# castacks/mvs_gi

Hardware: AMD Instinct MI355X
Metric: stereo frames/sec/GPU (G16V, 3-cam, D=16) + inv-dist L1 vs reference (higher is better)
Workload: dtype f16x3 (split-fp16 MFMA operands: 11 + 11 significant bits, f32 accumulate/activations)

## Files before the change

### include/mvsgi.h

```cpp
#ifndef MVSGI_H
#define MVSGI_H

#include <stddef.h>
#include <stdint.h>

#ifdef __cplusplus
extern "C" {
#endif

#define MVSGI_ABI_VERSION 8

typedef void* mvsgi_stream_t;

#define MVSGI_CONV_AUTO   0
#define MVSGI_CONV_DIRECT 1
#define MVSGI_CONV_MFMA   2
#define MVSGI_CONV_BF16X3 3
#define MVSGI_CONV_BF16X3_C16 4
#define MVSGI_CONV_BF16X3_V32 5
#define MVSGI_CONV_BF16X3_D32 6

#define MVSGI_CONV_F16 0x100

#define MVSGI_SPLIT_F16 1

int         mvsgi_abi_version(void);
const char* mvsgi_last_error(void);

#define MVSGI_SAT_SWEEP 1u
#define MVSGI_SAT_SPLIT 2u
#define MVSGI_SAT_WINO  4u
int mvsgi_saturation_flags(int clear, unsigned* flags);
int mvsgi_saturation_words(unsigned* words8);

int mvsgi_sweep_max_cams(void);
int mvsgi_sweep_std_f32(const float* feats, const float* grids, const void* grid_masks,
                        int grid_mask_is_f32, const float* masks, float* vol,
                        int B, int N, int C, int Hi, int Wi, int Hm, int Wm,
                        int D, int Ho, int Wo, mvsgi_stream_t stream);

int mvsgi_sweep_cat_f32(const float* feats, const float* grids, float* vol,
                        int B, int N, int C, int Hi, int Wi,
                        int D, int Ho, int Wo, mvsgi_stream_t stream);

int mvsgi_sweep_std_nhwc_f32(const float* feats, const float* grids, const void* grid_masks,
                             int grid_mask_is_f32, const float* masks, float* vol,
                             int B, int N, int C, int Hi, int Wi, int Hm, int Wm,
                             int D, int Ho, int Wo, mvsgi_stream_t stream);
int mvsgi_sweep_cat_nhwc_f32(const float* feats, const float* grids, float* vol,
                             int B, int N, int C, int Hi, int Wi,
                             int D, int Ho, int Wo, mvsgi_stream_t stream);

int mvsgi_sweep_validity_u8(const float* grids, const void* grid_masks, int grid_mask_is_f32,
                            const float* masks, unsigned char* vmask,
                            int B, int N, int Hm, int Wm, int D, int Ho, int Wo, mvsgi_stream_t stream);
int mvsgi_sweep_std_nhwc_valid_f32(const float* feats, const float* grids, const unsigned char* vmask,
                                   float* vol, int B, int N, int C, int Hi, int Wi,
                                   int D, int Ho, int Wo, mvsgi_stream_t stream);
int mvsgi_sweep_std_nhwc_valid_rig_f32(const float* feats, const float* grids, const unsigned char* vmask,
                                       float* vol, int B, int N, int C, int Hi, int Wi, int D, int Ho, int Wo,
                                       mvsgi_stream_t stream);

size_t mvsgi_conv3d_packed_weight_floats(int Cout, int Cin);
int mvsgi_conv3d_pack_weights_f32(const float* w_oidhw, float* w_packed, int Cout, int Cin,
                                  mvsgi_stream_t stream);
size_t mvsgi_conv3d_packed_weight_bytes_bf16x3(int Cout, int Cin);
int mvsgi_conv3d_pack_weights_bf16x3(const float* w_oidhw, void* w_packed, int Cout, int Cin,
                                     mvsgi_stream_t stream);
int mvsgi_conv3d_pack_weights_split(const float* w_oidhw, void* w_packed, int Cout, int Cin, int layout, mvsgi_stream_t stream);
int mvsgi_conv3d_f32(const float* x, const float* w_oidhw, const float* w_packed,
                     const float* scale, const float* shift, const float* res, float* y,
                     int B, int Cin, int Din, int Hin, int Win, int Cout,
                     int stride, float neg_slope, int impl, mvsgi_stream_t stream);
const char* mvsgi_conv3d_variant_f32(int B, int Cin, int Din, int Hin, int Win, int Cout,
                                     int stride, int impl);

int mvsgi_conv3d_up2_f32(const float* x, const void* w_packed, int w_layout ,
                         const float* scale, const float* shift, const float* res, float* y,
                         int B, int Cin, int Dl, int Hl, int Wl, int Cout, float neg_slope, mvsgi_stream_t stream);
const char* mvsgi_conv3d_up2_variant_f32(int B, int Cin, int Dl, int Hl, int Wl, int Cout, int w_layout);
int mvsgi_conv3d_v32_applies(int B, int Cin, int Din, int Hin, int Win, int Cout, int stride);
int mvsgi_conv3d_d32_applies(int B, int Cin, int Din, int Hin, int Win, int Cout, int stride);
int mvsgi_conv3d_up2_d32_applies(int B, int Cin, int Dl, int Hl, int Wl, int Cout);
size_t mvsgi_conv3d_packed_weight_bytes_bf16x3_v32(int Cout, int Cin);
int mvsgi_conv3d_pack_weights_bf16x3_v32(const float* w_oidhw, void* w_packed, int Cout, int Cin, mvsgi_stream_t stream);
size_t mvsgi_conv3d_packed_weight_bytes_bf16x3_c16(int Cin);
int mvsgi_conv3d_pack_weights_bf16x3_c16(const float* w_oidhw, void* w_packed, int Cin, mvsgi_stream_t stream);

size_t mvsgi_conv2d_packed_weight_floats(int Cout, int Cin);
int mvsgi_conv2d_pack_weights_f32(const float* w_oihw, float* w_packed, int Cout, int Cin,
                                  mvsgi_stream_t stream);
size_t mvsgi_conv2d_stem_packed_weight_bytes(void);
int mvsgi_conv2d_stem_pack_weights(const float* w_oihw, void* w_packed, mvsgi_stream_t stream);
size_t mvsgi_conv2d_packed_weight_bytes_bf16x3(int Cout, int Cin);
int mvsgi_conv2d_pack_weights_bf16x3(const float* w_oihw, void* w_packed, int Cout, int Cin,
                                     mvsgi_stream_t stream);
int mvsgi_conv2d_f32(const float* x, const float* w_oihw, const void* w_packed,
                     const float* scale, const float* shift, const float* res, float* y,
                     int B, int Cin, int Hin, int Win, int Cout, int ksize, int stride,
                     float neg_slope, int impl, int in_nchw, mvsgi_stream_t stream);
const char* mvsgi_conv2d_variant_f32(int Cin, int Cout, int ksize, int stride, int impl, int in_nchw);

int mvsgi_resize_trilinear_f32(const float* x, float* y, int B, int C,
                               int Di, int Hi, int Wi, int Do, int Ho, int Wo,
                               mvsgi_stream_t stream);

int mvsgi_softargmin_f32(const float* costs, const float* inv_idx, float* inv_dist,
                         float* norm_costs, int B, int D, int H, int W, int scale,
                         mvsgi_stream_t stream);

int mvsgi_softargmin_div_f32(const float* costs, const float* inv_idx, float* inv_dist,
                             float* norm_costs, int B, int D, int H, int W, int scale,
                             float post_div, mvsgi_stream_t stream);

#define MVSGI_SA_AUTO  0
#define MVSGI_SA_PIXEL 1
#define MVSGI_SA_BAND  2
int mvsgi_softargmin_scaled_f32(const float* costs, const float* inv_idx, float* inv_dist,
                                float* norm_costs, int B, int D, int H, int W, double scale,
                                int OH, int OW, float post_div, int variant, mvsgi_stream_t stream);

int mvsgi_confidence_f32(const float* costs, const float* inv_idx, float* max_prob, float* entropy,
                         float* spread, int* argmax, int B, int D, int H, int W, double scale,
                         int OH, int OW, float post_div, int normalize_entropy, mvsgi_stream_t stream);

int mvsgi_ncv_to_nvc_f32(const float* x, float* y, int B, int C, long long V, mvsgi_stream_t stream);
int mvsgi_nvc_to_ncv_f32(const float* x, float* y, int B, int C, long long V, mvsgi_stream_t stream);

int mvsgi_resblock2d_f32(const float* x, const void* w_packed1, const float* scale1, const float* shift1,
                         const void* w_packed2, const float* scale2, const float* shift2, float* y,
                         int N, int H, int W, float neg_slope, mvsgi_stream_t stream);

size_t mvsgi_split2d_bytes(int N, int H, int W);
int mvsgi_f32_to_split2d(const float* x, void* y_split, int N, int H, int W, mvsgi_stream_t stream);
int mvsgi_split2d_to_f32(const void* x_split, float* y, int N, int H, int W, mvsgi_stream_t stream);
size_t mvsgi_resblock2d_split_packed_weight_bytes(void);
int mvsgi_resblock2d_split_pack_weights(const float* w_oihw, const float* scale, void* w_packed, mvsgi_stream_t stream);
int mvsgi_resblock2d_split(const void* x_split, const void* w_packed1, const float* shift1,
                           const void* w_packed2, const float* shift2, void* y, int y_is_split,
                           int N, int H, int W, float neg_slope, mvsgi_stream_t stream);
int mvsgi_conv2d_s2_split(const void* x_split, const void* w_packed, const float* shift, void* y_split,
                          int N, int H, int W, float neg_slope, mvsgi_stream_t stream);
int mvsgi_conv2d_f32_out_split2d(const float* x, const float* w_oihw, const void* w_packed,
                                 const float* scale, const float* shift, const float* res, void* y_split,
                                 int B, int Cin, int Hin, int Win, int Cout, int ksize, int stride,
                                 float neg_slope, int impl, int in_nchw, mvsgi_stream_t stream);

int mvsgi_rays_panorama_f32(const float* dist, float* rays, int N, int H, int W,
                            float lat0, float lat1, float lon0, float lon1, mvsgi_stream_t stream);
int mvsgi_transform_points_f32(const float* T , const float* points, float* out,
                               int B, long long M, mvsgi_stream_t stream);
int mvsgi_grid_double_sphere_f32(const float* points, float* grid, unsigned char* mask, int B, long long M,
                                 float xi, float alpha, float fx, float fy, float cx, float cy,
                                 int calib_h, int calib_w, float w2, mvsgi_stream_t stream);
int mvsgi_grid_equirect_f32(const float* points, float* grid, int B, long long M, mvsgi_stream_t stream);
int mvsgi_rays_equirect_surrogate_f32(float* rays, int H, int W, mvsgi_stream_t stream);

int mvsgi_resample_bilinear_u8_f32(const unsigned char* imgs, const float* grid, const unsigned char* valid, float* out,
                                   long long M, int T, int Hr, int Wr, int H, int W, float invalid_value, mvsgi_stream_t stream);
int mvsgi_resample_bilinear_f32(const float* imgs, const float* grid, const unsigned char* valid, float* out, long long M, int T,
                                int C, int Hr, int Wr, int H, int W, float invalid_value, mvsgi_stream_t stream);
int mvsgi_resample_validity_u8(const float* grid, const unsigned char* ds_mask, unsigned char* valid, long long n,
                               mvsgi_stream_t stream);
int mvsgi_resample_u8_table_f32(float* table256);

int mvsgi_reproject_f32(const float* inv, const float* rays, const void* imgs, int img_kind, const float* T_host,
// ... 163 lines not shown
```

### mvs_gi_amd/_lib.py

```python
from __future__ import annotations

import ctypes
import os
from ctypes import c_char_p, c_double, c_float, c_int, c_longlong, c_size_t, c_void_p

_HERE = os.path.dirname(os.path.abspath(__file__))
LIB_PATH = os.environ.get("MVSGI_LIB", os.path.join(_HERE, "libmvsgi_hip.so"))

ABI_VERSION = 8


class MvsgiLibraryMissing(RuntimeError):
    pass


_P = c_void_p
SIGNATURES = {
    "mvsgi_abi_version": (c_int, []),
    "mvsgi_last_error": (c_char_p, []),
    "mvsgi_saturation_flags": (c_int, [c_int, _P]),
    "mvsgi_saturation_words": (c_int, [_P]),
    "mvsgi_sweep_max_cams": (c_int, []),
    "mvsgi_sweep_std_f32": (c_int, [_P, _P, _P, c_int, _P, _P] + [c_int] * 10 + [_P]),
    "mvsgi_sweep_cat_f32": (c_int, [_P, _P, _P] + [c_int] * 8 + [_P]),
    "mvsgi_sweep_std_nhwc_f32": (c_int, [_P, _P, _P, c_int, _P, _P] + [c_int] * 10 + [_P]),
    "mvsgi_sweep_cat_nhwc_f32": (c_int, [_P, _P, _P] + [c_int] * 8 + [_P]),
    "mvsgi_sweep_validity_u8": (c_int, [_P, _P, c_int, _P, _P] + [c_int] * 7 + [_P]),
    "mvsgi_sweep_std_nhwc_valid_f32": (c_int, [_P, _P, _P, _P] + [c_int] * 8 + [_P]),
    "mvsgi_sweep_std_nhwc_valid_split": (c_int, [_P, _P, _P, _P] + [c_int] * 9 + [_P]),
    "mvsgi_sweep_std_nhwc_valid_rig_f32": (c_int, [_P, _P, _P, _P] + [c_int] * 8 + [_P]),
    "mvsgi_conv3d_packed_weight_floats": (c_size_t, [c_int, c_int]),
    "mvsgi_conv3d_pack_weights_f32": (c_int, [_P, _P, c_int, c_int, _P]),
    "mvsgi_conv3d_packed_weight_bytes_bf16x3": (c_size_t, [c_int, c_int]),
    "mvsgi_conv3d_pack_weights_bf16x3": (c_int, [_P, _P, c_int, c_int, _P]),
    "mvsgi_conv3d_pack_weights_split": (c_int, [_P, _P, c_int, c_int, c_int, _P]),
    "mvsgi_conv3d_f32": (c_int, [_P] * 7 + [c_int] * 7 + [c_float, c_int, _P]),
    "mvsgi_conv3d_variant_f32": (c_char_p, [c_int] * 8),
    "mvsgi_conv3d_up2_f32": (c_int, [_P, _P, c_int] + [_P] * 4 + [c_int] * 6 + [c_float, _P]),
    "mvsgi_conv3d_up2_variant_f32": (c_char_p, [c_int] * 7),
    "mvsgi_conv3d_v32_applies": (c_int, [c_int] * 7),
    "mvsgi_conv3d_d32_applies": (c_int, [c_int] * 7),
    "mvsgi_conv3d_up2_d32_applies": (c_int, [c_int] * 6),
    "mvsgi_conv3d_packed_weight_bytes_bf16x3_v32": (c_size_t, [c_int, c_int]),
    "mvsgi_conv3d_pack_weights_bf16x3_v32": (c_int, [_P, _P, c_int, c_int, _P]),
    "mvsgi_conv3d_packed_weight_bytes_bf16x3_c16": (c_size_t, [c_int]),
    "mvsgi_conv3d_pack_weights_bf16x3_c16": (c_int, [_P, _P, c_int, _P]),
    "mvsgi_conv2d_stem_packed_weight_bytes": (c_size_t, []),
    "mvsgi_conv2d_stem_pack_weights": (c_int, [_P, _P, _P]),
    "mvsgi_conv2d_packed_weight_floats": (c_size_t, [c_int, c_int]),
    "mvsgi_conv2d_pack_weights_f32": (c_int, [_P, _P, c_int, c_int, _P]),
    "mvsgi_conv2d_packed_weight_bytes_bf16x3": (c_size_t, [c_int, c_int]),
    "mvsgi_conv2d_pack_weights_bf16x3": (c_int, [_P, _P, c_int, c_int, _P]),
    "mvsgi_conv2d_f32": (c_int, [_P] * 7 + [c_int] * 7 + [c_float, c_int, c_int, _P]),
    "mvsgi_conv2d_variant_f32": (c_char_p, [c_int] * 6),
    "mvsgi_resblock2d_f32": (c_int, [_P] * 8 + [c_int] * 3 + [c_float, _P]),
    "mvsgi_split2d_bytes": (c_size_t, [c_int] * 3),
    "mvsgi_f32_to_split2d": (c_int, [_P, _P] + [c_int] * 3 + [_P]),
    "mvsgi_split2d_to_f32": (c_int, [_P, _P] + [c_int] * 3 + [_P]),
    "mvsgi_resblock2d_split_packed_weight_bytes": (c_size_t, []),
    "mvsgi_resblock2d_split_pack_weights": (c_int, [_P, _P, _P, _P]),
    "mvsgi_resblock2d_split": (c_int, [_P] * 6 + [c_int] * 4 + [c_float, _P]),
    "mvsgi_conv2d_s2_split": (c_int, [_P] * 4 + [c_int] * 3 + [c_float, _P]),
    "mvsgi_conv2d_f32_out_split2d": (c_int, [_P] * 7 + [c_int] * 7 + [c_float, c_int, c_int, _P]),
    "mvsgi_resize_trilinear_f32": (c_int, [_P, _P] + [c_int] * 8 + [_P]),
    "mvsgi_softargmin_f32": (c_int, [_P, _P, _P, _P] + [c_int] * 5 + [_P]),
    "mvsgi_softargmin_div_f32": (c_int, [_P, _P, _P, _P] + [c_int] * 5 + [c_float, _P]),
    "mvsgi_softargmin_scaled_f32": (c_int, [_P, _P, _P, _P] + [c_int] * 4 + [c_double, c_int, c_int, c_float, c_int, _P]),
    "mvsgi_confidence_f32": (c_int, [_P] * 6 + [c_int] * 4 + [c_double, c_int, c_int, c_float, c_int, _P]),
    "mvsgi_rays_panorama_f32": (c_int, [_P, _P, c_int, c_int, c_int] + [c_float] * 4 + [_P]),
    "mvsgi_transform_points_f32": (c_int, [_P, _P, _P, c_int, c_longlong, _P]),
    "mvsgi_grid_double_sphere_f32": (c_int, [_P, _P, _P, c_int, c_longlong] + [c_float] * 6 + [c_int, c_int, c_float, _P]),
    "mvsgi_grid_equirect_f32": (c_int, [_P, _P, c_int, c_longlong, _P]),
    "mvsgi_rays_equirect_surrogate_f32": (c_int, [_P, c_int, c_int, _P]),
    "mvsgi_resample_bilinear_u8_f32": (c_int, [_P, _P, _P, _P, c_longlong] + [c_int] * 5 + [c_float, _P]),
    "mvsgi_resample_bilinear_f32": (c_int, [_P, _P, _P, _P, c_longlong] + [c_int] * 6 + [c_float, _P]),
    "mvsgi_resample_validity_u8": (c_int, [_P, _P, _P, c_longlong, _P]),
    "mvsgi_resample_u8_table_f32": (c_int, [_P]),
    "mvsgi_reproject_f32": (c_int, [_P, _P, _P, c_int] + [_P] * 6 + [c_longlong] + [c_int] * 6 + [c_float, c_float, _P]),
    "mvsgi_deform_conv2d_pack_weights_f32": (c_int, [_P, _P] + [c_int] * 4 + [_P]),
    "mvsgi_deform_conv2d_f32": (c_int, [_P, _P, c_int] + [_P] * 5 + [c_int] * 13 + [c_float, _P]),
    "mvsgi_act_split_bytes": (c_size_t, [c_int] * 5),
    "mvsgi_act_f32_to_split": (c_int, [_P, _P] + [c_int] * 5 + [_P]),
    "mvsgi_act_split_to_f32": (c_int, [_P, _P] + [c_int] * 5 + [_P]),
    "mvsgi_conv3d_f32_out_split": (c_int, [_P] * 6 + [c_int] * 7 + [c_float, _P]),
    "mvsgi_conv3d_rs16_split": (c_int, [_P] * 5 + [c_int] * 4 + [c_float, _P]),
    "mvsgi_conv3d_rs16_split_out_split": (c_int, [_P] * 5 + [c_int] * 4 + [c_float, _P]),
    "mvsgi_conv3d_s2rs_packed_weight_bytes": (c_size_t, []),
    "mvsgi_conv3d_s2rs_pack_weights": (c_int, [_P, _P, _P, _P]),
    "mvsgi_conv3d_s2rs": (c_int, [_P] * 4 + [c_int] * 4 + [c_float, _P]),
    "mvsgi_conv3d_rs_packed_weight_bytes": (c_size_t, [c_int, c_int]),
    "mvsgi_conv3d_rs_pack_weights": (c_int, [_P, _P, c_int, c_int, _P]),
    "mvsgi_conv3d_rs_split": (c_int, [_P] * 6 + [c_int] * 7 + [c_float, _P]),
    "mvsgi_conv3d_up2_f32_out_split": (c_int, [_P, _P, c_int] + [_P] * 4 + [c_int] * 6 + [c_float, _P]),
    "mvsgi_conv3d_up2_poly_split": (c_int, [_P] * 5 + [c_int] * 4 + [c_float, _P]),
    "mvsgi_conv3d_head_split_packed_weight_bytes": (c_size_t, [c_int]),
    "mvsgi_conv3d_head_split_pack_weights": (c_int, [_P, _P, c_int, _P]),
    "mvsgi_conv3d_head_split": (c_int, [_P, _P, c_float, c_float, _P] + [c_int] * 5 + [c_float, _P]),
    "mvsgi_conv3d_head_split_pack_weights_f16": (c_int, [_P, _P, c_int, _P]),
    "mvsgi_conv3d_head_split_f16": (c_int, [_P, _P, c_float, c_float, _P] + [c_int] * 5 + [c_float, _P]),
    "mvsgi_conv3d_head_rec32_f16": (c_int, [_P, _P, c_float, c_float, _P] + [c_int] * 5 + [c_float, _P]),
    "mvsgi_conv3d_up2_poly_rec32": (c_int, [_P] * 5 + [c_int] * 4 + [c_float, _P]),
    "mvsgi_conv3d_up2_poly_plan_bytes": (c_size_t, [c_int] * 3),
    "mvsgi_conv3d_up2_poly_plan": (c_int, [_P, _P] + [c_int] * 3),
    "mvsgi_conv3d_up2_poly_f32": (c_int, [_P] * 5 + [c_int] * 4 + [c_float, _P]),
    "mvsgi_act_f32_to_split_fmt": (c_int, [_P, _P] + [c_int] * 6 + [_P]),
    "mvsgi_act_split_to_f32_fmt": (c_int, [_P, _P] + [c_int] * 6 + [_P]),
    "mvsgi_sweep_std_nhwc_valid_split_fmt": (c_int, [_P, _P, _P, _P] + [c_int] * 10 + [_P]),
    "mvsgi_conv3d_f32_out_split_fmt": (c_int, [_P] * 6 + [c_int] * 7 + [c_float, c_int, _P]),
    "mvsgi_conv3d_rs_pack_weights_fmt": (c_int, [_P, _P, c_int, c_int, c_int, _P]),
    "mvsgi_conv3d_rs_split_fmt": (c_int, [_P] * 6 + [c_int] * 7 + [c_float, c_int, _P]),
    "mvsgi_conv3d_rs16_split_fmt": (c_int, [_P] * 5 + [c_int] * 5 + [c_float, c_int, _P]),
    "mvsgi_conv3d_s2rs_pack_weights_fmt": (c_int, [_P, _P, _P, c_int, _P]),
    "mvsgi_conv3d_s2rs_fmt": (c_int, [_P] * 4 + [c_int] * 4 + [c_float, c_float, c_int, _P]),
    "mvsgi_conv3d_s2rs_out_fmt": (c_int, [_P] * 4 + [c_int] * 4 + [c_float, c_float, c_int, c_int, _P]),
    "mvsgi_conv3d_up2_poly_plan_fmt": (c_int, [_P, _P] + [c_int] * 4),
    "mvsgi_conv3d_wino32_packed_weight_bytes": (c_size_t, []),
    "mvsgi_conv3d_wino32_applies": (c_int, [c_int] * 6 + [c_float]),
    "mvsgi_conv3d_wino32_pack_weights": (c_int, [_P] * 4),
    "mvsgi_conv3d_wino32_f16": (c_int, [_P] * 6 + [c_int] * 6 + [c_float, _P]),
    "mvsgi_conv3d_up2_poly_fmt": (c_int, [_P] * 5 + [c_int] * 5 + [c_float, c_int, _P]),
    "mvsgi_conv3d_up2_poly_wino_pays": (c_int, [c_int] * 4),
    "mvsgi_ncv_to_nvc_f32": (c_int, [_P, _P, c_int, c_int, c_longlong, _P]),
    "mvsgi_nvc_to_ncv_f32": (c_int, [_P, _P, c_int, c_int, c_longlong, _P]),
    "mvsgi_instance_norm_ws_bytes": (c_size_t, [c_int] * 3),
    "mvsgi_instance_norm_f32": (c_int, [_P] * 6 + [c_int] * 3 + [c_float, c_float, _P]),
# ... 60 lines not shown
```

### mvs_gi_amd/csrc/conv3d.hip

```cpp
#include "common.hpp"
#include "conv_common.hpp"
#include "conv3d_variants.hpp"
#ifdef MVSGI_STAMPS
#include <cstdio>
#include <cstdlib>
#endif

namespace {

__global__ void pack_head_weights_kernel(const float* __restrict__ w, float* __restrict__ wp, int Cin) {
    const int idx = blockIdx.x * 256 + threadIdx.x;
    if (idx >= 27 * Cin) return;
    const int tap = idx / Cin, ci = idx % Cin;
    wp[idx] = w[ci * 27 + tap];
}

#include "conv3d_f32mfma.hpp"
#include "conv3d_bf16x3.hpp"


__global__ __launch_bounds__(256) void conv3d_head_kernel(ConvArgs a, int dchunk, int nd) {
    constexpr int TH = 8, TW = 32, ITH = TH + 2, ITW = TW + 2, PV = ITH * ITW;
    constexpr int NT = (PV + 31) / 32;
    constexpr int TPW = (NT + 3) / 4;
// ... 139 lines not shown
__global__ __launch_bounds__(256) void conv3d_direct_kernel(ConvArgs a) {
    const int groups = (a.Cout + CO - 1) / CO;
    const long long total = (long long)a.B * a.Do * a.Ho * a.Wo * groups;
    const long long idx = (long long)blockIdx.x * 256 + threadIdx.x;
    if (idx >= total) return;
    const int cg = (int)(idx % groups);
    const long long vox = idx / groups;
    const int ow = (int)(vox % a.Wo);
    const int oh = (int)((vox / a.Wo) % a.Ho);
    const int od = (int)((vox / ((long long)a.Wo * a.Ho)) % a.Do);
    const int b = (int)(vox / ((long long)a.Wo * a.Ho * a.Do));
    const int co0 = cg * CO;
    float acc[CO];
#pragma unroll
    for (int o = 0; o < CO; ++o) acc[o] = 0.f;
    for (int kd = 0; kd < 3; ++kd) {
        const int id = od * a.stride - 1 + kd;
        if (id < 0 || id >= a.Din) continue;
        for (int kh = 0; kh < 3; ++kh) {
            const int ih = oh * a.stride - 1 + kh;
            if (ih < 0 || ih >= a.Hin) continue;
            for (int kw = 0; kw < 3; ++kw) {
                const int iw = ow * a.stride - 1 + kw;
                if (iw < 0 || iw >= a.Win) continue;
                const int tap = (kd * 3 + kh) * 3 + kw;
                const float* xp = a.x + ((((long long)b * a.Din + id) * a.Hin + ih) * a.Win + iw) * a.Cin;
                for (int ci = 0; ci < a.Cin; ++ci) {
                    const float xv = xp[ci];
#pragma unroll
                    for (int o = 0; o < CO; ++o) {
                        const int co = co0 + o;
                        if (co < a.Cout) acc[o] = fmaf(xv, a.w_oidhw[((long long)co * a.Cin + ci) * 27 + tap], acc[o]);
                    }
                }
            }
        }
    }
#pragma unroll
    for (int o = 0; o < CO; ++o) {
        const int co = co0 + o;
        if (co >= a.Cout) break;
        float r = acc[o] * a.scale[co] + a.shift[co];
        if (a.res) r += a.res[vox * a.Cout + co];
        r = r > 0.f ? r : r * a.neg_slope;
        a.y[vox * a.Cout + co] = r;
    }
}

int launch_head(ConvArgs a, hipStream_t st) {
    constexpr size_t lds_bytes = (size_t)27 * 360 * sizeof(float);
    a.tiles_h = (int)mvsgi::cdiv(a.Ho, 8);
    a.tiles_w = (int)mvsgi::cdiv(a.Wo, 32);
    const long long windows = (long long)a.B * a.tiles_h * a.tiles_w;
    long long nd = windows >= 1024 ? 1 : mvsgi::cdiv(1024, windows);
    if (nd > mvsgi::cdiv(a.Do, 2)) nd = mvsgi::cdiv(a.Do, 2);
    const int dchunk = (int)mvsgi::cdiv(a.Do, nd);
    nd = mvsgi::cdiv(a.Do, dchunk);
    a.tiles_d = (int)nd;
    const long long nt = windows * nd;
    MVSGI_REQUIRE(nt < (1ll << 31), "conv3d: too many tiles");
    MVSGI_REQUIRE((long long)a.Hin * a.Win * a.Cin < (1ll << 31), "conv3d(head): plane too large for 32-bit offsets");
    hipLaunchKernelGGL(conv3d_head_kernel, dim3((unsigned)nt), dim3(256), lds_bytes, st, a, dchunk, (int)nd);
    return mvsgi::check_launch("mvsgi_conv3d_f32(head)");
}

int launch_direct(const ConvArgs& a, hipStream_t st) {
    const long long vox = (long long)a.B * a.Do * a.Ho * a.Wo;
    if (a.Cout == 1) {
        hipLaunchKernelGGL((conv3d_direct_kernel<1>), dim3((unsigned)mvsgi::cdiv(vox, 256)), dim3(256), 0, st, a);
    } else {
        const long long total = vox * mvsgi::cdiv(a.Cout, 4);
        hipLaunchKernelGGL((conv3d_direct_kernel<4>), dim3((unsigned)mvsgi::cdiv(total, 256)), dim3(256), 0, st, a);
    }
    return mvsgi::check_launch("mvsgi_conv3d_f32(direct)");
}

bool v32_applies(const ConvArgs& a) {
    if (a.Cout % 32 || a.Cin % 16 || a.stride != 1) return false;
    const long long big = (long long)a.B * mvsgi::cdiv(a.Do, 4) * mvsgi::cdiv(a.Ho, 4) * mvsgi::cdiv(a.Wo, 16);
    const long long mid = (long long)a.B * mvsgi::cdiv(a.Do, 2) * mvsgi::cdiv(a.Ho, 4) * mvsgi::cdiv(a.Wo, 16);
    return a.Cout == 32 ? big >= 384 : mid * mvsgi::cdiv(a.Cout, 64) >= 384;
}

int select_variant_up2(const ConvArgs& a, int w_layout) {
    if (w_layout == MVSGI_CONV_BF16X3_D32) {
        const int base = a.Cin % 32 ? V_COUNT : select_variant_up2(a, MVSGI_CONV_BF16X3);
        const bool d2 = a.Do == 2;
        if (base == B3U_N64) return d2 ? B3DU2_N64 : B3DU_N64;
        if (base == B3U_N96) return d2 ? B3DU2_N96 : B3DU_N96;
        mvsgi::fail("mvsgi_conv3d_up2_f32: the 32-channel-slice kernels do not apply to this problem (see mvsgi_conv3d_up2_d32_applies)");
        return V_COUNT;
    }
    const bool c16_layout = w_layout == MVSGI_CONV_BF16X3_C16;
    if (w_layout == MVSGI_CONV_BF16X3_V32) {
        if (!v32_applies(a) || !a.wp) { mvsgi::fail("mvsgi_conv3d_up2_f32: the 32x32x16 kernel does not apply to this problem"); return V_COUNT; }
        return a.Cout == 32 ? B3VU_N32 : B3VU_N64;
    }
    if (a.Cin % 16 || a.Cout % 16) {
        mvsgi::fail("mvsgi_conv3d_up2_f32: Cin, Cout must be multiples of 16 (got %d, %d)", a.Cin, a.Cout);
        return V_COUNT;
    }
    if (!a.wp) { mvsgi::fail("mvsgi_conv3d_up2_f32: needs w_packed (bf16x3 layout)"); return V_COUNT; }
    const int CT = a.Cout / 16;
    const long long big = (long long)a.B * mvsgi::cdiv(a.Do, 4) * mvsgi::cdiv(a.Ho, 4) * mvsgi::cdiv(a.Wo, 16);
    const long long mid = (long long)a.B * mvsgi::cdiv(a.Do, 2) * mvsgi::cdiv(a.Ho, 4) * mvsgi::cdiv(a.Wo, 16);
    if (CT == 1) return c16_layout ? B3PU_N16 : B3U_N16;
    if (CT == 2) {
        if (big >= 384) return B3U_N32;
        const long long cus = mvsgi::device_cus(), r32 = mvsgi::cdiv(big, cus), rm = mvsgi::cdiv(mid, cus);
        return 157 * (100 + 85 * (r32 - 1)) < 100 * (100 + 85 * (rm - 1)) ? B3U_N32 : B3U_N32_M;
    }
    if (CT == 3) return B3U_N48;
    if (CT % 6 == 0 && mid * (CT / 6) >= 384) return B3U_N96;
    if (CT % 2 == 0 && (long long)a.B * mvsgi::cdiv(a.Do, 2) * mvsgi::cdiv(a.Ho, 2) * mvsgi::cdiv(a.Wo, 16) * (CT / 2) <= mvsgi::device_cus())
        return B3U_N32_TB;
    return B3U_N64;
}

int select_variant(const ConvArgs& a, int impl);

int d32_variant(const ConvArgs& a) {
    if (a.stride != 1 || a.Cin % 32 || a.Cout % 16) return V_COUNT;
    ConvArgs b = a;
    static const float dummy = 0.f;
    if (!b.wp) b.wp = reinterpret_cast<const f32x4*>(&dummy);
    const bool d2 = a.Do == 2;
    switch (select_variant(b, MVSGI_CONV_BF16X3)) {
        case B3_N64: return d2 ? B3D2_N64 : B3D_N64;
        case B3_N64_H5: return d2 ? B3D2_N64_H5 : B3D_N64_H5;
        case B3_N64_W8: return d2 ? B3D2_N64_W8 : B3D_N64_W8;
        case B3_N96: return d2 ? B3D2_N96 : B3D_N96;
        case B3_N96_H5: return d2 ? B3D2_N96_H5 : B3D_N96_H5;
        case B3_N96_W8: return d2 ? B3D2_N96_W8 : B3D_N96_W8;
        case B3_N128_P: return B3D_N128_P;
        case B3_N128_PH5: return B3D_N128_PH5;
        case B3_N128_PW8: return B3D_N128_PW8;
        case B3_N192_PH5: return B3D_N192_PH5;
        case B3_N192_PW8: return B3D_N192_PW8;
        case B3_N16_TW: return d2 && a.Cout % 32 == 0 ? B3D2_N32_TB : V_COUNT;
        case B3_N32_TB: return d2 ? B3D2_N32_TB : B3D_N32_TB;
        case B3_N64_S: return d2 ? B3D2_N64_S : B3D_N64_S;
        default: return V_COUNT;
    }
}

int select_variant(const ConvArgs& a, int impl) {
    const bool mfma_ok = (a.Cin % 16 == 0) && (a.Cout % 16 == 0);
    const bool head_ok = (a.Cout == 1) && (a.Cin % 16 == 0) && (a.stride == 1);
    if (impl == MVSGI_CONV_BF16X3_C16) {
        if (a.Cout != 16 || a.Cin % 16 || a.stride != 1) {
            mvsgi::fail("mvsgi_conv3d_f32: the Cout == 16 plane kernel needs Cout == 16, Cin %% 16 == 0, stride 1 (got %d, %d, %d)",
                        a.Cout, a.Cin, a.stride);
            return V_COUNT;
        }
        if (!a.wp) { mvsgi::fail("mvsgi_conv3d_f32: tiled path needs w_packed"); return V_COUNT; }
        return B3P_N16;
    }
    if (impl == MVSGI_CONV_BF16X3_V32) {
        if (!v32_applies(a)) {
            mvsgi::fail("mvsgi_conv3d_f32: the 32x32x16 kernel does not apply to this problem (see mvsgi_conv3d_v32_applies)");
            return V_COUNT;
        }
        if (!a.wp) { mvsgi::fail("mvsgi_conv3d_f32: tiled path needs w_packed"); return V_COUNT; }
        return a.Cout == 32 ? B3V_N32 : B3V_N64;
    }
    if (impl == MVSGI_CONV_BF16X3_D32) {
        const int v = d32_variant(a);
// ... 12 lines not shown
        return V_COUNT;
    }
    if (!a.wp) { mvsgi::fail("mvsgi_conv3d_f32: tiled path needs w_packed"); return V_COUNT; }
    if (head_ok && impl == MVSGI_CONV_MFMA) return V_HEAD;
    if (!mfma_ok) {
        mvsgi::fail("mvsgi_conv3d_f32: MFMA path needs Cin, Cout multiples of 16 (got %d, %d)", a.Cin, a.Cout);
        return V_COUNT;
    }
    const int CT = a.Cout / 16;
    const long long vox = (long long)a.B * a.Do * a.Ho * a.Wo;
    if (impl == MVSGI_CONV_BF16X3) {
        if (a.stride == 2) {
            const long long s2bricks = (long long)a.B * mvsgi::cdiv(a.Do, 2) * mvsgi::cdiv(a.Ho, 4) * mvsgi::cdiv(a.Wo, 8);
            if (CT % 12 == 0 && s2bricks * (CT / 12) >= 512) return B3_S2_N192;
            if (CT % 8 == 0 && s2bricks * (CT / 8) >= 512) return B3_S2_N128;
            if (CT % 6 == 0 && s2bricks * (CT / 6) >= 512) return B3_S2_N96;
            if (CT <= 3 || s2bricks * mvsgi::cdiv(CT, 2) <= mvsgi::device_cus()) return B3_S2_N32B;
            return B3_S2_N64;
        }
        const long long big = (long long)a.B * mvsgi::cdiv(a.Do, 4) * mvsgi::cdiv(a.Ho, 4) * mvsgi::cdiv(a.Wo, 16);
        const long long mid = (long long)a.B * mvsgi::cdiv(a.Do, 2) * mvsgi::cdiv(a.Ho, 4) * mvsgi::cdiv(a.Wo, 16);
        if (CT == 1) return B3_N16;
        if (CT == 2) return big >= 384 ? B3_N32 : B3_N32_TB;
        if (CT == 3) return B3_N48;
        const bool h5ok = a.Ho % 5 == 0 && a.Ho % 4 != 0;
        const bool w8 = a.Ho % 10 == 0 && a.Wo % 16 == 8;
        if (a.Do == 1 && CT >= 8 && CT % 4 == 0) {
            const long long rows5 = (long long)a.B * (a.Ho / 5) * mvsgi::cdiv(a.Wo, 16);
            if (h5ok && CT % 12 == 0 && rows5 * (CT / 12) >= 384) return w8 ? B3_N192_PW8 : B3_N192_PH5;
            if (h5ok && CT % 8 == 0 && rows5 * (CT / 8) >= mvsgi::device_cus() / 2) return w8 ? B3_N128_PW8 : B3_N128_PH5;
            if (CT % 8 == 0 && (long long)a.B * mvsgi::cdiv(a.Ho, 4) * mvsgi::cdiv(a.Wo, 16) * (CT / 8) >= 384) return B3_N128_P;
        }
        if (CT % 6 == 0 && h5ok &&
            (long long)a.B * mvsgi::cdiv(a.Do, 2) * (a.Ho / 5) * mvsgi::cdiv(a.Wo, 16) * (CT / 6) >= 384) return w8 ? B3_N96_W8 : B3_N96_H5;
        if (CT % 6 == 0 && mid * (CT / 6) >= 384) return B3_N96;
        const long long cus = mvsgi::device_cus();
        if (CT % 4 == 0 && CT % 6 != 0 && mid * (CT / 4) < 4 * cus) {
            const long long tiny = (long long)a.B * a.Do * mvsgi::cdiv(a.Ho, 4) * mvsgi::cdiv(a.Wo, 16);
            if (tiny * CT <= cus) return B3_N16_TW;
            const long long slices = a.Cin / 16;
            struct Cand { int v; long long units, a_ns, b_ns; };
            const Cand cand[] = {
                {B3_N32_TB, tiny * (CT / 2), 5700, 1000},
                {B3_N64_S, tiny * (CT / 4), 6600, 1700},
                {B3_N64, mid * (CT / 4), 8700, 2600},
                {w8 ? B3_N64_W8 : B3_N64_H5, a.Ho % 5 ? 0 : (long long)a.B * mvsgi::cdiv(a.Do, 2) * (CT / 4) *
                                                 (w8 ? (a.Ho / 10) * (a.Wo / 8) : (a.Ho / 5) * mvsgi::cdiv(a.Wo, 16)), 8400, 3500},
            };
            int best = B3_N64;
            long long best_cost = -1;
            for (const Cand& c : cand) {
                if (c.units <= 0) continue;
                const long long rounds = mvsgi::cdiv(c.units, cus);
                const long long cost = (c.a_ns + c.b_ns * slices) * (100 + 85 * (rounds - 1));
                if (best_cost < 0 || cost < best_cost) { best_cost = cost; best = c.v; }
            }
            return best;
        }
        if (h5ok && (long long)a.B * mvsgi::cdiv(a.Do, 2) * (a.Ho / 5) * mvsgi::cdiv(a.Wo, 16) * mvsgi::cdiv(CT, 4) >= 384)
            return w8 ? B3_N64_W8 : B3_N64_H5;
        if (mid * mvsgi::cdiv(CT, 4) >= 384) return B3_N64;
        const long long tiny = (long long)a.B * a.Do * mvsgi::cdiv(a.Ho, 4) * mvsgi::cdiv(a.Wo, 16);
        if (tiny * CT <= cus) return B3_N16_TW;
        const long long rounds32 = mvsgi::cdiv(tiny * mvsgi::cdiv(CT, 2), cus), rounds64 = mvsgi::cdiv(tiny * mvsgi::cdiv(CT, 4), cus);
        return 2 * rounds32 <= 3 * rounds64 ? B3_N32_TB : B3_N64_S;
    }
    if (a.stride == 1) {
        if (CT == 1) return V_S1_N16_B256;
        if (CT <= 3) return vox >= 256ll * 512 ? V_S1_N32_B256 : V_S1_N32_B64;
        return vox * CT >= 128ll * 4 * 1024 ? V_S1_N64_B128 : V_S1_N64_B64;
    }
    return CT <= 3 ? V_S2_N32_B64 : V_S2_N64_B64;
}

int launch_variant(int v, const ConvArgs& a, hipStream_t st) {
    if (a.f16) return mvsgi::conv3d_launch_b3_f16(v, &a, st);
    switch (v) {
        case V_DIRECT1:
        case V_DIRECT4: return launch_direct(a, st);
        case V_HEAD: return launch_head(a, st);
#define MVSGI_MFMA(V, ...) case V: return launch_mfma<__VA_ARGS__>(a, st);
#define MVSGI_B3(V, K, ...) case V: return MVSGI_B3_LAUNCH##K(false, __VA_ARGS__)(a, st);
#include "conv3d_variants.inc"
#undef MVSGI_MFMA
#undef MVSGI_B3
    }
    return mvsgi::fail("mvsgi_conv3d_f32: bad variant %d", v);
}

int fill_args(ConvArgs& a, const float* x, const float* w_oidhw, const float* w_packed, const float* scale,
              const float* shift, const float* res, float* y, int B, int Cin, int Din, int Hin, int Win, int Cout,
              int stride, float neg_slope) {
    MVSGI_REQUIRE(B > 0 && Cin > 0 && Cout > 0 && Din > 0 && Hin > 0 && Win > 0, "mvsgi_conv3d_f32: bad dims");
    MVSGI_REQUIRE(stride == 1 || stride == 2, "mvsgi_conv3d_f32: stride %d not in {1, 2}", stride);
    a.x = x;
    a.w_oidhw = w_oidhw;
    a.wp = reinterpret_cast<const f32x4*>(w_packed);
    a.scale = scale;
    a.shift = shift;
    a.res = res;
    a.y = y;
    a.B = B;
    a.Cin = Cin;
    a.Din = Din;
    a.Hin = Hin;
    a.Win = Win;
    a.Cout = Cout;
    a.stride = stride;
    a.neg_slope = neg_slope;
    a.Do = (Din - 1) / stride + 1;
    a.Ho = (Hin - 1) / stride + 1;
    a.Wo = (Win - 1) / stride + 1;
    return 0;
}

int split_flag(ConvArgs& a, int& impl, const char* who) {
    a.f16 = (impl & MVSGI_CONV_F16) != 0;
    impl &= ~MVSGI_CONV_F16;
    MVSGI_REQUIRE(!a.f16 || impl == MVSGI_CONV_BF16X3 || impl == MVSGI_CONV_BF16X3_C16 || impl == MVSGI_CONV_BF16X3_V32 || impl == MVSGI_CONV_BF16X3_D32,
                  "%s: MVSGI_CONV_F16 goes with MVSGI_CONV_BF16X3 / _C16 / _V32 (got %d)", who, impl);
    MVSGI_REQUIRE(!a.f16 || (a.Cin % 16 == 0 && a.Cout % 16 == 0), "%s: the fp16 split needs Cin, Cout multiples of 16 (got %d, %d)", who, a.Cin, a.Cout);
    return 0;
}

const char* variant_name(int v, const ConvArgs& a) {
    switch (v) {
        case V_DIRECT1: return "conv3d_direct_kernel<1>";
        case V_DIRECT4: return "conv3d_direct_kernel<4>";
        case V_HEAD: return "conv3d_head_kernel";
#define MVSGI_MFMA(V, ...) case V: return "conv3d_mfma_kernel<" #__VA_ARGS__ ">";
#define MVSGI_B3(V, K, ...) case V: return a.f16 ? "conv3d_f16x3" #K "<" #__VA_ARGS__ ">" : "conv3d_bf16x3" #K "<" #__VA_ARGS__ ">";
#include "conv3d_variants.inc"
#undef MVSGI_MFMA
#undef MVSGI_B3
    }
    return nullptr;
}

}

extern "C" size_t mvsgi_conv3d_packed_weight_floats(int Cout, int Cin) {
    return (size_t)27 * (size_t)Cout * (size_t)Cin;
}

extern "C" size_t mvsgi_conv3d_packed_weight_bytes_bf16x3(int Cout, int Cin) {
    return (size_t)(Cin / 16) * pairs_of(3) * (size_t)(Cout / 16) * 2 * 64 * 16;
}

extern "C" int mvsgi_conv3d_pack_weights_bf16x3(const float* w_oidhw, void* w_packed, int Cout, int Cin,
                                                mvsgi_stream_t stream) {
    MVSGI_REQUIRE(w_oidhw && w_packed, "mvsgi_conv3d_pack_weights_bf16x3: null pointer");
    MVSGI_REQUIRE(Cout > 0 && Cin > 0 && Cout % 16 == 0 && Cin % 16 == 0,
                  "mvsgi_conv3d_pack_weights_bf16x3: Cout=%d Cin=%d must be positive multiples of 16", Cout, Cin);
    const long long total = (long long)(Cin / 16) * pairs_of(3) * (Cout / 16) * 64;
    hipLaunchKernelGGL(pack_weights_bf16x3_kernel, dim3((unsigned)mvsgi::cdiv(total, 256)), dim3(256), 0,
                       mvsgi::as_stream(stream), w_oidhw, reinterpret_cast<bf16x8*>(w_packed), Cout, Cin, 27, false);
    return mvsgi::check_launch("mvsgi_conv3d_pack_weights_bf16x3");
}

extern "C" int mvsgi_conv3d_pack_weights_split(const float* w_oidhw, void* w_packed, int Cout, int Cin, int layout,
                                               mvsgi_stream_t stream) {
    MVSGI_REQUIRE(w_oidhw && w_packed, "mvsgi_conv3d_pack_weights_split: null pointer");
    const bool f16 = (layout & MVSGI_CONV_F16) != 0;
    layout &= ~MVSGI_CONV_F16;
    MVSGI_REQUIRE(Cout > 0 && Cin > 0 && Cout % 16 == 0 && Cin % 16 == 0,
                  "mvsgi_conv3d_pack_weights_split: Cout=%d Cin=%d must be positive multiples of 16", Cout, Cin);
    bf16x8* wp = reinterpret_cast<bf16x8*>(w_packed);
    if (layout == MVSGI_CONV_BF16X3) {
        const long long total = (long long)(Cin / 16) * pairs_of(3) * (Cout / 16) * 64;
        hipLaunchKernelGGL(pack_weights_bf16x3_kernel, dim3((unsigned)mvsgi::cdiv(total, 256)), dim3(256), 0, mvsgi::as_stream(stream),
                           w_oidhw, wp, Cout, Cin, 27, f16);
    } else if (layout == MVSGI_CONV_BF16X3_C16) {
        MVSGI_REQUIRE(Cout == 16, "mvsgi_conv3d_pack_weights_split: the plane layout is for Cout == 16 (got %d)", Cout);
        const int total = (Cin / 16) * 5 * 3 * 64;
        hipLaunchKernelGGL(pack_weights_bf16x3_c16_kernel, dim3((unsigned)mvsgi::cdiv(total, 256)), dim3(256), 0, mvsgi::as_stream(stream),
                           w_oidhw, wp, Cin, f16);
    } else if (layout == MVSGI_CONV_BF16X3_V32) {
        MVSGI_REQUIRE(Cout % 32 == 0, "mvsgi_conv3d_pack_weights_split: the 32x32x16 layout needs Cout %% 32 == 0 (got %d)", Cout);
        const long long total = (long long)(Cin / 16) * (Cout / 32) * 27 * 64;
        hipLaunchKernelGGL(pack_weights_bf16x3_v32_kernel, dim3((unsigned)mvsgi::cdiv(total, 256)), dim3(256), 0, mvsgi::as_stream(stream),
                           w_oidhw, wp, Cout, Cin, f16);
    } else if (layout == MVSGI_CONV_BF16X3_D32) {
        MVSGI_REQUIRE(Cin % 32 == 0, "mvsgi_conv3d_pack_weights_split: the 32-channel-slice layout needs Cin %% 32 == 0 (got %d)", Cin);
        const long long total = (long long)(Cin / 32) * (Cout / 16) * 27 * 64;
        const size_t used = (size_t)total * 2 * sizeof(bf16x8), all = mvsgi_conv3d_packed_weight_bytes_bf16x3(Cout, Cin);
        MVSGI_REQUIRE(used <= all && hipMemsetAsync(reinterpret_cast<char*>(w_packed) + used, 0, all - used, mvsgi::as_stream(stream)) == hipSuccess,
                      "mvsgi_conv3d_pack_weights_split: clearing the unused tail of the 32-channel-slice layout failed");
        hipLaunchKernelGGL(pack_weights_bf16x3_d32_kernel, dim3((unsigned)mvsgi::cdiv(total, 256)), dim3(256), 0, mvsgi::as_stream(stream),
                           w_oidhw, wp, Cout, Cin, f16);
    } else {
        return mvsgi::fail("mvsgi_conv3d_pack_weights_split: layout %d is not a split-kernel layout", layout);
    }
    return mvsgi::check_launch("mvsgi_conv3d_pack_weights_split");
}

extern "C" size_t mvsgi_conv3d_packed_weight_bytes_bf16x3_v32(int Cout, int Cin) {
    return (size_t)(Cin / 16) * (Cout / 32) * 27 * 2 * 64 * 16;
}

extern "C" int mvsgi_conv3d_pack_weights_bf16x3_v32(const float* w_oidhw, void* w_packed, int Cout, int Cin,
                                                    mvsgi_stream_t stream) {
    MVSGI_REQUIRE(w_oidhw && w_packed, "mvsgi_conv3d_pack_weights_bf16x3_v32: null pointer");
    MVSGI_REQUIRE(Cout > 0 && Cin > 0 && Cout % 32 == 0 && Cin % 16 == 0,
                  "mvsgi_conv3d_pack_weights_bf16x3_v32: Cout=%d must be a multiple of 32, Cin=%d of 16", Cout, Cin);
    const long long total = (long long)(Cin / 16) * (Cout / 32) * 27 * 64;
    hipLaunchKernelGGL(pack_weights_bf16x3_v32_kernel, dim3((unsigned)mvsgi::cdiv(total, 256)), dim3(256), 0,
                       mvsgi::as_stream(stream), w_oidhw, reinterpret_cast<bf16x8*>(w_packed), Cout, Cin, false);
    return mvsgi::check_launch("mvsgi_conv3d_pack_weights_bf16x3_v32");
}

extern "C" int mvsgi_conv3d_d32_applies(int B, int Cin, int Din, int Hin, int Win, int Cout, int stride) {
    ConvArgs a{};
    static const float dummy = 0.f;
    if (fill_args(a, &dummy, &dummy, &dummy, &dummy, &dummy, nullptr, nullptr, B, Cin, Din, Hin, Win, Cout, stride, 1.f))
        return 0;
    return d32_variant(a) != V_COUNT ? 1 : 0;
}

extern "C" int mvsgi_conv3d_v32_applies(int B, int Cin, int Din, int Hin, int Win, int Cout, int stride) {
    ConvArgs a{};
    static const float dummy = 0.f;
    if (fill_args(a, &dummy, &dummy, &dummy, &dummy, &dummy, nullptr, nullptr, B, Cin, Din, Hin, Win, Cout, stride, 1.f))
        return 0;
    return v32_applies(a) ? 1 : 0;
}

extern "C" size_t mvsgi_conv3d_packed_weight_bytes_bf16x3_c16(int Cin) { return (size_t)(Cin / 16) * 5 * 3 * 2 * 64 * 16; }

extern "C" int mvsgi_conv3d_pack_weights_bf16x3_c16(const float* w_oidhw, void* w_packed, int Cin, mvsgi_stream_t stream) {
    MVSGI_REQUIRE(w_oidhw && w_packed, "mvsgi_conv3d_pack_weights_bf16x3_c16: null pointer");
    MVSGI_REQUIRE(Cin > 0 && Cin % 16 == 0, "mvsgi_conv3d_pack_weights_bf16x3_c16: Cin=%d must be a positive multiple of 16", Cin);
    const int total = (Cin / 16) * 5 * 3 * 64;
    hipLaunchKernelGGL(pack_weights_bf16x3_c16_kernel, dim3((unsigned)mvsgi::cdiv(total, 256)), dim3(256), 0,
                       mvsgi::as_stream(stream), w_oidhw, reinterpret_cast<bf16x8*>(w_packed), Cin, false);
    return mvsgi::check_launch("mvsgi_conv3d_pack_weights_bf16x3_c16");
}

extern "C" int mvsgi_conv3d_pack_weights_f32(const float* w_oidhw, float* w_packed, int Cout, int Cin,
                                             mvsgi_stream_t stream) {
    MVSGI_REQUIRE(w_oidhw && w_packed, "mvsgi_conv3d_pack_weights_f32: null pointer");
    if (Cout == 1 && Cin > 0 && Cin % 16 == 0) {
        hipLaunchKernelGGL(pack_head_weights_kernel, dim3((unsigned)mvsgi::cdiv(27 * Cin, 256)), dim3(256), 0,
                           mvsgi::as_stream(stream), w_oidhw, w_packed, Cin);
        return mvsgi::check_launch("mvsgi_conv3d_pack_weights_f32");
    }
    MVSGI_REQUIRE(Cout > 0 && Cin > 0 && Cout % 16 == 0 && Cin % 16 == 0,
                  "mvsgi_conv3d_pack_weights_f32: Cout=%d Cin=%d must be positive multiples of 16 (or Cout == 1)",
                  Cout, Cin);
    const long long total = (long long)(Cin / 16) * 27 * (Cout / 16) * 64;
    hipLaunchKernelGGL(pack_weights_kernel, dim3((unsigned)mvsgi::cdiv(total, 256)), dim3(256), 0,
                       mvsgi::as_stream(stream), w_oidhw, reinterpret_cast<f32x4*>(w_packed), Cout, Cin, 27);
    return mvsgi::check_launch("mvsgi_conv3d_pack_weights_f32");
}

extern "C" int mvsgi_conv3d_f32(const float* x, const float* w_oidhw, const float* w_packed, const float* scale,
                                const float* shift, const float* res, float* y, int B, int Cin, int Din, int Hin,
                                int Win, int Cout, int stride, float neg_slope, int impl, mvsgi_stream_t stream) {
    MVSGI_REQUIRE(x && y && scale && shift, "mvsgi_conv3d_f32: null pointer");
    ConvArgs a{};
    if (fill_args(a, x, w_oidhw, w_packed, scale, shift, res, y, B, Cin, Din, Hin, Win, Cout, stride, neg_slope))
        return 1;
    if (split_flag(a, impl, "mvsgi_conv3d_f32")) return 1;
    const int v = select_variant(a, impl);
    if (v == V_COUNT) return 1;
    return launch_variant(v, a, mvsgi::as_stream(stream));
}

extern "C" int mvsgi_conv3d_f32_out_split_fmt(const float* x, const float* w_packed_b3, const float* scale, const float* shift,
                                              const float* res, void* y_split, int B, int Cin, int Din, int Hin, int Win, int Cout,
                                              int stride, float neg_slope, int fmt, mvsgi_stream_t stream) {
    MVSGI_REQUIRE(fmt == 0 || fmt == MVSGI_SPLIT_F16, "mvsgi_conv3d_f32_out_split: fmt %d not in {0, MVSGI_SPLIT_F16}", fmt);
    MVSGI_REQUIRE(x && y_split && scale && shift && w_packed_b3, "mvsgi_conv3d_f32_out_split: null pointer");
    MVSGI_REQUIRE(Cin % 16 == 0 && Cout % 16 == 0, "mvsgi_conv3d_f32_out_split: Cin, Cout must be multiples of 16");
    ConvArgs a{};
    if (fill_args(a, x, nullptr, w_packed_b3, scale, shift, res, reinterpret_cast<float*>(y_split), B, Cin, Din, Hin, Win, Cout,
                  stride, neg_slope))
        return 1;
    a.y_split = static_cast<unsigned char*>(y_split);
    a.f16 = fmt != 0;
    const int v = select_variant(a, MVSGI_CONV_BF16X3);
    if (v == V_COUNT) return 1;
    return launch_variant(v, a, mvsgi::as_stream(stream));
}
extern "C" int mvsgi_conv3d_f32_out_split(const float* x, const float* w_packed_b3, const float* scale, const float* shift,
                                          const float* res, void* y_split, int B, int Cin, int Din, int Hin, int Win, int Cout,
                                          int stride, float neg_slope, mvsgi_stream_t stream) {
    return mvsgi_conv3d_f32_out_split_fmt(x, w_packed_b3, scale, shift, res, y_split, B, Cin, Din, Hin, Win, Cout, stride, neg_slope, 0, stream);
}

extern "C" const char* mvsgi_conv3d_variant_f32(int B, int Cin, int Din, int Hin, int Win, int Cout, int stride,
                                                int impl) {
    ConvArgs a{};
    static const float dummy = 0.f;
    if (fill_args(a, &dummy, &dummy, &dummy, &dummy, &dummy, nullptr, nullptr, B, Cin, Din, Hin, Win, Cout, stride,
                  1.f))
        return nullptr;
    if (split_flag(a, impl, "mvsgi_conv3d_variant_f32")) return nullptr;
    const int v = select_variant(a, impl);
    return variant_name(v, a);
}

extern "C" int mvsgi_conv3d_up2_f32(const float* x, const void* w_packed, int w_layout, const float* scale,
                                    const float* shift, const float* res, float* y, int B, int Cin, int Dl, int Hl,
                                    int Wl, int Cout, float neg_slope, mvsgi_stream_t stream) {
    const bool f16 = (w_layout & MVSGI_CONV_F16) != 0;
    w_layout &= ~MVSGI_CONV_F16;
    MVSGI_REQUIRE(w_layout == MVSGI_CONV_BF16X3 || (w_layout == MVSGI_CONV_BF16X3_C16 && Cout == 16) ||
                      (w_layout == MVSGI_CONV_BF16X3_V32 && Cout % 32 == 0) || (w_layout == MVSGI_CONV_BF16X3_D32 && Cin % 32 == 0),
                  "mvsgi_conv3d_up2_f32: w_layout %d not valid for Cout %d", w_layout, Cout);
    MVSGI_REQUIRE(x && y && scale && shift && w_packed, "mvsgi_conv3d_up2_f32: null pointer");
    MVSGI_REQUIRE(Dl > 0 && Hl > 0 && Wl > 0 && Dl < (1 << 20) && Hl < (1 << 20) && Wl < (1 << 20),
                  "mvsgi_conv3d_up2_f32: bad dims");
    ConvArgs a{};
    if (fill_args(a, x, nullptr, static_cast<const float*>(w_packed), scale, shift, res, y, B, Cin, 2 * Dl, 2 * Hl,
                  2 * Wl, Cout, 1, neg_slope))
        return 1;
    a.f16 = f16;
    const int v = select_variant_up2(a, w_layout);
    if (v == V_COUNT) return 1;
    return launch_variant(v, a, mvsgi::as_stream(stream));
}

extern "C" int mvsgi_conv3d_up2_f32_out_split(const float* x, const void* w_packed, int w_layout, const float* scale, const float* shift,
                                              const float* res, void* y_split, int B, int Cin, int Dl, int Hl, int Wl, int Cout,
                                              float neg_slope, mvsgi_stream_t stream) {
    const bool f16 = (w_layout & MVSGI_CONV_F16) != 0;
    w_layout &= ~MVSGI_CONV_F16;
    MVSGI_REQUIRE(w_layout == MVSGI_CONV_BF16X3 || (w_layout == MVSGI_CONV_BF16X3_C16 && Cout == 16),
                  "mvsgi_conv3d_up2_f32_out_split: w_layout %d not valid for Cout %d", w_layout, Cout);
    MVSGI_REQUIRE(x && y_split && scale && shift && w_packed, "mvsgi_conv3d_up2_f32_out_split: null pointer");
    MVSGI_REQUIRE(Dl > 0 && Hl > 0 && Wl > 0 && Dl < (1 << 20) && Hl < (1 << 20) && Wl < (1 << 20),
                  "mvsgi_conv3d_up2_f32_out_split: bad dims");
    ConvArgs a{};
    if (fill_args(a, x, nullptr, static_cast<const float*>(w_packed), scale, shift, res, reinterpret_cast<float*>(y_split), B, Cin,
                  2 * Dl, 2 * Hl, 2 * Wl, Cout, 1, neg_slope))
        return 1;
    a.y_split = static_cast<unsigned char*>(y_split);
    a.f16 = f16;
    const int v = select_variant_up2(a, w_layout);
    if (v == V_COUNT) return 1;
    return launch_variant(v, a, mvsgi::as_stream(stream));
}

extern "C" int mvsgi_conv3d_up2_d32_applies(int B, int Cin, int Dl, int Hl, int Wl, int Cout) {
    ConvArgs a{};
    static const float dummy = 0.f;
    if (Cin % 32 || Cout % 16 || Dl <= 0 || Hl <= 0 || Wl <= 0 ||
        fill_args(a, &dummy, nullptr, &dummy, &dummy, &dummy, nullptr, nullptr, B, Cin, 2 * Dl, 2 * Hl, 2 * Wl, Cout, 1, 1.f))
        return 0;
    const int base = select_variant_up2(a, MVSGI_CONV_BF16X3);
    return (base == B3U_N64 || base == B3U_N96) ? 1 : 0;
}

extern "C" const char* mvsgi_conv3d_up2_variant_f32(int B, int Cin, int Dl, int Hl, int Wl, int Cout, int w_layout) {
    ConvArgs a{};
    static const float dummy = 0.f;
    if (fill_args(a, &dummy, nullptr, &dummy, &dummy, &dummy, nullptr, nullptr, B, Cin, 2 * Dl, 2 * Hl, 2 * Wl, Cout, 1,
                  1.f))
        return nullptr;
    a.f16 = (w_layout & MVSGI_CONV_F16) != 0;
    const int v = select_variant_up2(a, w_layout & ~MVSGI_CONV_F16);
    return variant_name(v, a);
}
```

### mvs_gi_amd/csrc/conv3d_bf16x3.hpp

```cpp
#pragma once
#ifndef MVSGI_ABL
#define MVSGI_ABL 0
#endif

#include "split_fmt.hpp"

constexpr int kVSB = 80;

__device__ __forceinline__ void split_bf16x4(const f32x4 x, u32x2& hi, u32x2& lo) {
#pragma unroll
    for (int p = 0; p < 2; ++p) {
        const f32x2 v = {x[2 * p], x[2 * p + 1]};
        const unsigned hb = __builtin_bit_cast(unsigned, __builtin_convertvector(v, bf16x2));
        const f32x2 hf = {__builtin_bit_cast(float, hb << 16), __builtin_bit_cast(float, hb & 0xffff0000u)};
        hi[p] = hb;
        float r0 = v[0] - hf[0], r1 = v[1] - hf[1];
        asm volatile("" : "+v"(r0));
        asm volatile("" : "+v"(r1));
        lo[p] = __builtin_bit_cast(unsigned, __builtin_convertvector(f32x2{r0, r1}, bf16x2));
    }
}
__device__ __forceinline__ f32x4 fma4(const f32x4 a, const f32x4 b, const f32x4 c) {
    f32x4 r;
#pragma unroll
// ... 81 lines not shown
    const long long o = ((((long long)cc * CT + ct) * kPairs + p) * 2) * 64 + lane;
    wp[o] = __builtin_bit_cast(bf16x8, hi);
    wp[o + 64] = __builtin_bit_cast(bf16x8, lo);
}

__global__ void pack_weights_bf16x3_d32_kernel(const float* __restrict__ w, bf16x8* __restrict__ wp, int Cout, int Cin, bool f16 = false) {
    const int CT = Cout / 16;
    const long long total = (long long)(Cin / 32) * CT * 27 * 64;
    const long long idx = (long long)blockIdx.x * 256 + threadIdx.x;
    if (idx >= total) return;
    const int lane = (int)(idx & 63);
    long long r = idx >> 6;
    const int tap = (int)(r % 27);
    r /= 27;
    const int ct = (int)(r % CT);
    const int cc = (int)(r / CT);
    const int kg = lane >> 4;
    const int co = ct * 16 + (lane & 15);
    const int ci = (2 * cc + (kg & 1)) * 16 + (kg >> 1) * 8;
    u16x8 hi, lo;
    for (int j = 0; j < 8; ++j) {
        unsigned short h_, l_;
        split_weight(w[((long long)co * Cin + ci + j) * 27 + tap], f16, h_, l_);
        hi[j] = h_;
        lo[j] = l_;
    }
    const long long o = ((((long long)cc * CT + ct) * 27 + tap) * 2) * 64 + lane;
    wp[o] = __builtin_bit_cast(bf16x8, hi);
    wp[o + 64] = __builtin_bit_cast(bf16x8, lo);
}

__global__ void pack_weights_bf16x3_c16_kernel(const float* __restrict__ w, bf16x8* __restrict__ wp, int Cin, bool f16 = false) {
    const int total = (Cin / 16) * 5 * 3 * 64;
    const int idx = blockIdx.x * 256 + threadIdx.x;
    if (idx >= total) return;
    const int lane = idx & 63;
    int r = idx >> 6;
    const int kd = r % 3;
    r /= 3;
    const int p = r % 5;
    const int cc = r / 5;
    const int kg = lane >> 4, co = lane & 15;
    const int ci = cc * 16 + (kg >> 1) * 8;
    const int t2 = 2 * p + (kg & 1);
    u16x8 hi, lo;
    for (int j = 0; j < 8; ++j) {
        const float v = t2 < 9 ? w[((long long)co * Cin + ci + j) * 27 + kd * 9 + t2] : 0.f;
        unsigned short h_, l_;
        split_weight(v, f16, h_, l_);
        hi[j] = h_;
        lo[j] = l_;
    }
    const long long o = ((long long)((cc * 5 + p) * 3 + kd) * 2) * 64 + lane;
    wp[o] = __builtin_bit_cast(bf16x8, hi);
    wp[o + 64] = __builtin_bit_cast(bf16x8, lo);
}

__global__ void pack_weights_bf16x3_v32_kernel(const float* __restrict__ w, bf16x8* __restrict__ wp, int Cout, int Cin, bool f16 = false) {
    const int CT = Cout / 32;
    const long long total = (long long)(Cin / 16) * CT * 27 * 64;
    const long long idx = (long long)blockIdx.x * 256 + threadIdx.x;
    if (idx >= total) return;
    const int lane = (int)(idx & 63);
    long long r = idx >> 6;
    const int tap = (int)(r % 27);
    r /= 27;
    const int ct = (int)(r % CT);
    const int cc = (int)(r / CT);
    const int co = ct * 32 + (lane & 31);
    const int ci = cc * 16 + (lane >> 5) * 8;
    u16x8 hi, lo;
    for (int j = 0; j < 8; ++j) {
        const float v = w[((long long)co * Cin + ci + j) * 27 + tap];
        unsigned short h_, l_;
        split_weight(v, f16, h_, l_);
        hi[j] = h_;
        lo[j] = l_;
    }
    const long long o = ((((long long)cc * CT + ct) * 27 + tap) * 2) * 64 + lane;
    wp[o] = __builtin_bit_cast(bf16x8, hi);
    wp[o + 64] = __builtin_bit_cast(bf16x8, lo);
}

template <int NW, int MW, int WM, int WN, int TD, int TH, int TW, int S, int KD, bool UPS, bool PLANE, bool V32, bool WLDS, bool F16, bool D32 = false, int DK = 3, int BRD = 0>
__device__ __forceinline__ void conv3d_x3_body(const ConvArgs& a) {
    static_assert(!WLDS || (WN == 1 && KD == 3 && !UPS && !PLANE && !V32 && S == 1 && NW == 1 && MW <= 2), "LDS-staged weights: one shared cout tile, one or two voxel tiles per wave");
    static_assert(!V32 || (S == 1 && KD == 3 && TW == 16 && TH % 2 == 0 && !PLANE), "32x32x16 schedule: stride 1, 16-wide even bricks");
    static_assert(!PLANE || (NW == 1 && WN == 1 && WM == 4 && TH == 4 && MW == TD && TW == 16 && S == 1 && KD == 3),
                  "plane schedule: Cout == 16, 4 h-rows x TD planes x 16 w per brick");
    static_assert(!UPS || (S == 1 && KD == 3 && TD % 2 == 0 && TH % 2 == 0 && TW % 2 == 0),
                  "fused upsample: stride 1, even bricks (halo bricks are whole 2x2x2 cells)");
    static_assert(WM * WN == 4, "4 consumer waves per workgroup");
    static_assert(WM * MW * (V32 ? 32 : 16) == TD * TH * TW, "brick must be covered by the voxel tiles");
    static_assert(KD == 3 || (KD == 1 && TD == 1), "2-D bricks are one plane thick");
    constexpr int SD = KD == 1 ? 1 : S;
    static_assert(!D32 || (KD == 3 && S == 1 && !PLANE && !V32 && !WLDS), "32-channel slices: stride-1 3x3x3 variants (plain or fused upsample) only");
    static_assert(DK == 3 || (D32 && DK >= 1 && (TD == 1 ? DK <= 2 : (TD == 2 && WM == 2 && MW * 16 == TH * TW))), "depth skip: one- or two-plane bricks whose waves own whole planes");
    constexpr bool DKU = D32 && TD == 1 && DK == 2;
    constexpr int kTaps = KD * 9, kPairs = D32 ? 9 * DK : pairs_of(KD);
    constexpr int kWBlk = D32 ? 27 : kPairs;
    constexpr int ITD = (TD - 1) * SD + KD, ITH = (TH - 1) * S + 3, ITW = (TW - 1) * S + 3;
    constexpr int IV = ITD * ITH * ITW;
    constexpr int QB = D32 ? 3 : 2;
    constexpr int NIT = (IV * (1 << QB) + 255) / 256;
    constexpr int ROWP = V32 ? ((ITW * kVSB + 255) / 256) * 256 : ITW * kVSB;
    constexpr int SUB = ITD * ITH * ROWP;
    constexpr int BUF = D32 ? 2 * SUB : SUB;
    constexpr int WB = WLDS ? (MW * NW == 1 ? 8 : 4) :
                       (KD == 3 && !PLANE && !V32 && MW * NW == 1) ? 16 : (KD == 3 && !PLANE && !V32 && MW * NW == 2) ? 8 :
                       (KD == 3 && !PLANE && !V32 && NW == 2 && MW == 4) ? 5 :
                       NW <= 2 ? 4 : 2;
    constexpr int LA = WB - 1;
    constexpr int NSLOT = ((kPairs + WB - 1) / WB) * WB;
    static_assert(NSLOT % WB == 0 && NSLOT >= kPairs, "pipeline geometry");
    constexpr bool RPRE = MW * NW <= 8;
#ifndef MVSGI_WARM
#define MVSGI_WARM 0
#endif
    constexpr bool WARM = MVSGI_WARM && KD == 3 && !UPS && !PLANE && !V32 && !WLDS && S == 1 && MW * NW <= 2;

    constexpr int WBYTES = WLDS ? NW * kPairs * 2048 : 0;
    constexpr int BUFW = BUF + WBYTES;
    constexpr int WARM_LDS = 2 * BUFW;
    extern __shared__ __attribute__((aligned(16))) unsigned char ldsb[];
    float satm = 0.f;

    const int tid = threadIdx.x, lane = tid & 63;
    const int wave = __builtin_amdgcn_readfirstlane(tid >> 6);
    const bool producer = wave >= 4;
    const int CT = a.Cout / (V32 ? 32 : 16);
    const int ny = (CT + WN * NW - 1) / (WN * NW);
    const int nchunks = a.Cin / (D32 ? 32 : 16);
    const int total = a.total_units;
    const int G = gridDim.x;
    const int nmine = (total - (int)blockIdx.x + G - 1) / G;
    const int U = nmine * nchunks;
#ifdef MVSGI_STAMPS
    int nst = 0;
#define STAMP()                                                                                     \
    if (a.dbg && blockIdx.x == 8 && nst < 120) {                                                    \
        unsigned long long t_;                                                                      \
        asm volatile("s_memtime %0\n\ts_waitcnt lgkmcnt(0)" : "=s"(t_)::"memory");                  \
        if (lane == 0) a.dbg[wave * 128 + nst] = t_;                                                \
        nst++;                                                                                      \
    }
#else
#define STAMP()
#endif
    STAMP()

#define MVSGI_DECODE_DH(T, OD, OH, B) { OD = (T % a.tiles_d) * TD + a.od_off; T /= a.tiles_d; OH = (T % a.tiles_h) * TH; B = T / a.tiles_h; }
#define MVSGI_DECODE(ID, CB, B, OD, OH, OW)                       \
    {                                                             \
        int t_ = xcd_remap((ID), total);                          \
        CB = t_ % ny;                                             \
        t_ /= ny;                                                 \
        OW = (t_ % a.tiles_w) * TW;                               \
        t_ /= a.tiles_w;                                          \
        MVSGI_DECODE_DH(t_, OD, OH, B)                            \
    }

    if (producer) {
        const int ptid = tid - 256;
        if constexpr (UPS) {
            constexpr int CD = ITD / 2, CH = ITH / 2, CW = ITW / 2, NC = CD * CH * CW;
            constexpr int NCQ = NC << QB;
            constexpr int NITU = (NCQ + 255) / 256;
            constexpr int RF = NCQ / 256, REM = NCQ - RF * 256;
            constexpr bool HALF = REM > 0 && 2 * REM <= 256;
#define MVSGI_UPS_CQ(IT) ((HALF && (IT) == RF) ? RF * 256 + (ptid >> 1) : ptid + (IT) * 256)
#define MVSGI_UPS_LIVE(IT) ((HALF && (IT) == RF) ? (ptid >> 1) < REM : ptid + (IT) * 256 < NCQ)
            const int Dl = a.Din >> 1, Hl = a.Hin >> 1, Wl = a.Win >> 1;
            const int sH_ = Wl * a.Cin, sD_ = Hl * sH_;
            int lo_d[NITU], lo_h[NITU], lo_w[NITU];
            unsigned inmask[NITU];
            const float* xb = a.x;
            f32x4 crA[NITU][8], crB[NITU][8];
            unsigned imA[NITU], imB[NITU];
#define MVSGI_PLAN_UPS(UNIT)                                                                            \
            {                                                                                           \
                int cb_, b_, od_, oh_, ow_;                                                             \
                MVSGI_DECODE(UNIT, cb_, b_, od_, oh_, ow_)                                              \
                (void)cb_;                                                                              \
                _Pragma("unroll") for (int it = 0; it < NITU; ++it) {                                   \
                    const int c = MVSGI_UPS_CQ(it) >> QB;                                               \
                    const int cw = c % CW, ch = (c / CW) % CH, cd = c / (CW * CH);                      \
                    const int gd = od_ - 1 + 2 * cd, gh = oh_ - 1 + 2 * ch, gw = ow_ - 1 + 2 * cw;      \
                    lo_d[it] = (gd - 1) >> 1;                                                           \
                    lo_h[it] = (gh - 1) >> 1;                                                           \
                    lo_w[it] = (gw - 1) >> 1;                                                           \
                    inmask[it] = (gd >= 0 && gd < a.Din ? 1u : 0u) | (gd + 1 < a.Din ? 2u : 0u) |       \
                                 (gh >= 0 && gh < a.Hin ? 4u : 0u) | (gh + 1 < a.Hin ? 8u : 0u) |       \
                                 (gw >= 0 && gw < a.Win ? 16u : 0u) | (gw + 1 < a.Win ? 32u : 0u);      \
                }                                                                                       \
                xb = a.x + (long long)b_ * Dl * Hl * Wl * a.Cin;                                        \
            }
#define MVSGI_CLAMP(V, N) ((V) < 0 ? 0 : ((V) > (N) - 1 ? (N) - 1 : (V)))
            int k2 = 0, cc2 = 0;
#define MVSGI_ISSUE_UPS_BEGIN()                                                                         \
            if (cc2 == 0 && k2 > 0) { MVSGI_PLAN_UPS((int)blockIdx.x + k2 * G) }
#define MVSGI_ISSUE_UPS1(CR, IM, IT)                                                                    \
            {                                                                                           \
                const int q = MVSGI_UPS_CQ(IT) & ((1 << QB) - 1);                                       \
                const bool live = MVSGI_UPS_LIVE(IT);                                                   \
                const int d0 = live ? MVSGI_CLAMP(lo_d[IT], Dl) : 0, d1 = live ? MVSGI_CLAMP(lo_d[IT] + 1, Dl) : 0; \
                const int h0 = live ? MVSGI_CLAMP(lo_h[IT], Hl) : 0, h1 = live ? MVSGI_CLAMP(lo_h[IT] + 1, Hl) : 0; \
                const int w0 = live ? MVSGI_CLAMP(lo_w[IT], Wl) : 0, w1 = live ? MVSGI_CLAMP(lo_w[IT] + 1, Wl) : 0; \
                const int cofs = cc2 * (D32 ? 32 : 16) + q * 4;                                         \
                 \
                const int od_[2] = {__mul24(d0, sD_), __mul24(d1, sD_)}, oh_[2] = {__mul24(h0, sH_), __mul24(h1, sH_)};   \
                const int ow_[2] = {__mul24(w0, a.Cin) + cofs, __mul24(w1, a.Cin) + cofs};              \
                _Pragma("unroll") for (int k = 0; k < 8; ++k)                                           \
                    CR[IT][k] = *reinterpret_cast<const f32x4*>(xb + (od_[(k >> 2) & 1] + oh_[(k >> 1) & 1] + ow_[k & 1])); \
                IM[IT] = inmask[IT];                                                                    \
            }
#define MVSGI_ISSUE_UPS_END()                                                                           \
            {                                                                                           \
                if (++cc2 == nchunks) { cc2 = 0; ++k2; }                                                \
                if (k2 >= nmine) { k2 = nmine - 1; cc2 = nchunks - 1; }                                 \
            }
#define MVSGI_ISSUE_UPS(CR, IM)                                                                         \
            {                                                                                           \
                MVSGI_ISSUE_UPS_BEGIN()                                                                 \
                _Pragma("unroll") for (int it = 0; it < NITU; ++it) MVSGI_ISSUE_UPS1(CR, IM, it)        \
                MVSGI_ISSUE_UPS_END()                                                                   \
            }
#define MVSGI_LERP2(A, B, O0, O1)    \
            {                                                                                           \
                const f32x4 d_ = fma4((A), f32x4{-1.f, -1.f, -1.f, -1.f}, (B));    \
                O0 = fma4(d_, f32x4{0.25f, 0.25f, 0.25f, 0.25f}, (A));             \
                O1 = fma4(d_, f32x4{0.75f, 0.75f, 0.75f, 0.75f}, (A));             \
            }
#define MVSGI_PUT_UPS1(CR, IM, DST, IT)                                                                 \
            if (HALF && (IT) == RF) {                                                                   \
                 \
                if (MVSGI_UPS_LIVE(IT)) {                                                               \
                    const int cq_ = MVSGI_UPS_CQ(IT), c = cq_ >> QB, q = cq_ & 3, kd = ptid & 1;        \
                    const int sub_ = D32 ? ((cq_ >> 2) & 1) * SUB : 0;                                  \
                    const int cw = c % CW, ch = (c / CW) % CH, cd = c / (CW * CH);                      \
                    const float f_ = kd ? 0.75f : 0.25f;                                                \
                    const f32x4 f4_ = {f_, f_, f_, f_};                                                 \
                    f32x4 xd[2][2], xh[2][2], xo[2][2];                                                 \
                    _Pragma("unroll") for (int j = 0; j < 4; ++j) {                                     \
                        const f32x4 d_ = fma4(CR[IT][j], f32x4{-1.f, -1.f, -1.f, -1.f}, CR[IT][4 + j]); \
                        xd[j >> 1][j & 1] = fma4(d_, f4_, CR[IT][j]);              \
                    }                                                                                   \
                    _Pragma("unroll") for (int kw = 0; kw < 2; ++kw)                                    \
// ... 328 lines not shown
            }
            MVSGI_V_READX(0, 0)
            if (XA == 2) { MVSGI_V_READX(1, 1) }
#pragma unroll
            for (int t_ = 0; t_ < 27; ++t_) {
                const int cur = t_ % VB, nx2 = (t_ + XA) % VB, wcur = t_ % VWB;
                unsigned l16 = lane16;
                asm volatile("" : "+v"(l16));
                if (t_ + LAW < 27) {
                    MVSGI_V_LOADW((t_ + LAW) % VWB, cc, t_ + LAW, ctc)
                } else {
                    MVSGI_V_LOADW((t_ + LAW - 27) % VWB, ncc, t_ + LAW - 27, ctn)
                }
                if (t_ + XA < 27) { MVSGI_V_READX(nx2, t_ + XA) }
                if (t_ == 26 && last && a.res) {
                    const float* rb = a.res + (long long)b_ * frame_elems;
#pragma unroll
                    for (int i = 0; i < MW; ++i)
#pragma unroll
                        for (int j = 0; j < NW; ++j)
#pragma unroll
                            for (int g = 0; g < 4; ++g)
                                rres[i][j][g] = *reinterpret_cast<const f32x4*>(rb + (eoff[i] >= 0 ? eoff[i] + ctc[j] * 32 + 8 * g : 0));
                }
                MVSGI_V_MFMAS(wcur, cur)
                if (t_ + XA < 27) {
                    constexpr int NMEM = 2 * NW + 2 * MW, NMFMA = 3 * MW * NW;
                    constexpr int RATIO = NMFMA / NMEM > 0 ? NMFMA / NMEM : 1;
#pragma unroll
                    for (int q_ = 0; q_ < NMEM; ++q_) {
                        __builtin_amdgcn_sched_group_barrier(0x008, RATIO, 0);
                        __builtin_amdgcn_sched_group_barrier(0x120, 1, 0);
                    }
                    __builtin_amdgcn_sched_group_barrier(0x008, NMFMA, 0);
                }
                __builtin_amdgcn_sched_barrier(0);
            }
            STAMP()
            if (last) {
                const int ct0 = (cb_ * WN + wn) * NW;
                float* yb = a.y + (long long)b_ * frame_elems;
#pragma unroll
                for (int i = 0; i < MW; ++i)
#pragma unroll
                    for (int j = 0; j < NW; ++j)
#pragma unroll
                        for (int g = 0; g < 4; ++g) {
                            f32x4 r = f32x4{acc[i][j][4 * g], acc[i][j][4 * g + 1], acc[i][j][4 * g + 2], acc[i][j][4 * g + 3]} * esc[j][g] + esh[j][g];
                            if (a.res) r += rres[i][j][g];
#pragma unroll
                            for (int e = 0; e < 4; ++e) {
                                r[e] = r[e] > 0.f ? r[e] : r[e] * a.neg_slope;
                                acc[i][j][4 * g + e] = 0.f;
                            }
                            if (eoff[i] >= 0 && ct0 + j < CT) *reinterpret_cast<f32x4*>(yb + eoff[i] + (ct0 + j) * 32 + 8 * g) = r;
                        }
                k += 1;
                cb_ = ncb; b_ = nb; od0 = nod0; oh0 = noh0; ow0 = now0;
#pragma unroll
                for (int j = 0; j < NW; ++j) ctc[j] = ctn[j];
            }
            cc = ncc;
            STAMP()
            __syncthreads();
            STAMP()
        }
#undef MVSGI_CTILES
#undef MVSGI_V_LOADW
#undef MVSGI_V_READX
#undef MVSGI_V_MFMAS
    } else {
        const int wm = wave % WM, wn = wave / WM;
        const int col = lane & 15, kg = lane >> 4;
        constexpr bool BSK = D32 && DK == 3 && TD == 2 && WM == 2 && MW == 4 && TH == 4 && TW == 16 && S == 1;
        static_assert(BRD == 0 || BSK, "border-plane skip: the 2 x 4 x 16 bricks of the 32-channel-slice kernels");
        const bool second = kg & 1;
        const char* wpb = reinterpret_cast<const char*>(a.wp);
        const unsigned lane16 = lane * 16;
        int base[MW];
#pragma unroll
        for (int i = 0; i < MW; ++i) {
            const int v = (wm * MW + i) * 16 + col;
            const int w_ = v % TW, h_ = BSK ? 2 * wm + (i & 1) : (v / TW) % TH, d_ = BSK ? (BRD == 2 ? 1 - (i >> 1) : (i >> 1)) : v / (TW * TH);
            base[i] = (((d_ * SD) * ITH + h_ * S) * ITW + w_ * S) * kVSB + (kg >> 1) * 16;
        }
        int tdv[MW], thv[MW], twv[MW];
#pragma unroll
        for (int i = 0; i < MW; ++i) {
            const int v = PLANE ? (i * TH + wm) * TW + col : (wm * MW + i) * 16 + col;
            twv[i] = v % TW;
            thv[i] = BSK ? 2 * wm + (i & 1) : (v / TW) % TH;
            tdv[i] = BSK ? (BRD == 2 ? 1 - (i >> 1) : (i >> 1)) : v / (TW * TH);
        }
        if constexpr (D32 && DK < 3 && !DKU) {
            const int kd_lo = (TD == 2 ? wm : 0) == 0 ? 1 : 0;
            wpb += kd_lo * 9 * 2048;
#pragma unroll
            for (int i = 0; i < MW; ++i) base[i] += kd_lo * (ITH * ITW * kVSB);
        }
        const long long frame_elems = (long long)a.Do * a.Ho * a.Wo * a.Cout;
        int ctc[NW], ctn[NW];
#define MVSGI_CTILES(DST, CB)                                                         \
        _Pragma("unroll") for (int j = 0; j < NW; ++j) {                              \
            const int c_ = ((CB) * WN + wn) * NW + j;                                 \
            DST[j] = c_ < CT ? c_ : CT - 1;                                           \
        }
        bf16x8 wh[WB][NW], wl[WB][NW];
        constexpr int XB = (KD == 3 && !PLANE && !V32 && MW * NW == 1) ? 8 : (KD == 3 && !PLANE && !V32 && MW * NW == 2) ? 4 : MW <= 4 ? 2 : 1;
        constexpr int XLA = XB > 1 ? XB - 1 : 1;
        constexpr int MH = XB >= 2 ? MW : MW / 2;
        bf16x8 xh[XB][MW], xl[XB][MW];
#define MVSGI_TAP(P) (BRD == 2 ? (2 - (P) / 9) * 9 + (P) % 9 : (P))
#define MVSGI_LOADW(BUFI, CC, P, CTS) MVSGI_LOADWB(wpb, BUFI, CC, P, CTS)
#define MVSGI_LOADWB(WPB, BUFI, CC, P, CTS)                                                           \
        _Pragma("unroll") for (int j = 0; j < NW; ++j) {                                              \
            const char* q_ = (WPB) + (((long long)(CC) * CT + CTS[j]) * kWBlk) * 2048;   \
            wh[BUFI][j] = *reinterpret_cast<const bf16x8*>(q_ + (l16 + (unsigned)MVSGI_TAP(P) * 2048u));          \
            wl[BUFI][j] = *reinterpret_cast<const bf16x8*>(q_ + (l16 + (unsigned)MVSGI_TAP(P) * 2048u + 1024u));  \
        }
#define MVSGI_READX(BUFI, P, I0, I1)                                                                  \
        {                                                                                             \
            const int p_ = (P);                                                                       \
            const int t0_ = 2 * p_, t1_ = (2 * p_ + 1 < kTaps) ? 2 * p_ + 1 : 2 * p_;                 \
            const int o0_ = (((t0_ / 9) * ITH + (t0_ / 3) % 3) * ITW + t0_ % 3) * kVSB;               \
            const int o1_ = (((t1_ / 9) * ITH + (t1_ / 3) % 3) * ITW + t1_ % 3) * kVSB;               \
            const int tp_ = MVSGI_TAP(p_);                                                            \
            const int od_ = (((tp_ / 9) * ITH + (tp_ / 3) % 3) * ITW + tp_ % 3) * kVSB;    \
            const int off_ = D32 ? od_ + (second ? SUB : 0) : (second ? o1_ : o0_);                   \
            _Pragma("unroll") for (int i = (I0); i < (I1); ++i) {                                     \
                xh[BUFI][i] = *reinterpret_cast<const bf16x8*>(img + base[i] + off_);                 \
                xl[BUFI][i] = *reinterpret_cast<const bf16x8*>(img + base[i] + off_ + 32);            \
            }                                                                                         \
            if constexpr (WLDS) {    \
                _Pragma("unroll") for (int j = 0; j < NW; ++j) {                                      \
                    wh[BUFI][j] = *reinterpret_cast<const bf16x8*>(img + BUF + (j * kPairs + p_) * 2048 + (int)lane16);          \
                    wl[BUFI][j] = *reinterpret_cast<const bf16x8*>(img + BUF + (j * kPairs + p_) * 2048 + 1024 + (int)lane16);   \
                }                                                                                     \
            }                                                                                         \
        }
#define MVSGI_MFMAS(WBUF, XBUF, I0, I1)                                                               \
        _Pragma("unroll") for (int i = (I0); i < (I1); ++i)                                           \
            _Pragma("unroll") for (int j = 0; j < NW; ++j)                                            \
                acc[i][j] = mfma16<F16>(wl[WBUF][j], xh[XBUF][i], acc[i][j]); \
        _Pragma("unroll") for (int i = (I0); i < (I1); ++i)                                           \
            _Pragma("unroll") for (int j = 0; j < NW; ++j)                                            \
                (TACC ? acc1[i][j] : acc[i][j]) = mfma16<F16>(wh[WBUF][j], xl[XBUF][i], TACC ? acc1[i][j] : acc[i][j]); \
        _Pragma("unroll") for (int i = (I0); i < (I1); ++i)                                           \
            _Pragma("unroll") for (int j = 0; j < NW; ++j)                                            \
                (TACC ? acc2[i][j] : acc[i][j]) = mfma16<F16>(wh[WBUF][j], xh[XBUF][i], TACC ? acc2[i][j] : acc[i][j]);
        constexpr bool TACC = KD == 3 && !PLANE && !V32 && MW * NW <= 2;
        f32x4 acc[MW][NW], acc1[MW][NW], acc2[MW][NW];
#pragma unroll
        for (int i = 0; i < MW; ++i)
#pragma unroll
            for (int j = 0; j < NW; ++j) {
                acc[i][j] = f32x4{0.f, 0.f, 0.f, 0.f};
                if (TACC) acc1[i][j] = acc2[i][j] = f32x4{0.f, 0.f, 0.f, 0.f};
            }

        int cb_, b_, od0, oh0, ow0;
        MVSGI_DECODE((int)blockIdx.x, cb_, b_, od0, oh0, ow0)
        MVSGI_CTILES(ctc, cb_)
        constexpr int NPP = 5;
        constexpr int PD = PLANE ? TD + 2 : 1;
        bf16x8 pwh[3][PLANE ? 3 : 1], pwl[3][PLANE ? 3 : 1];
        bf16x8 pxh[2][PD], pxl[2][PD];
        const int pbase = (wm * ITW + col) * kVSB + (kg >> 1) * 16;
#define MVSGI_PL_LOADW(BUFI, CC, P)                                                                    \
        _Pragma("unroll") for (int kd = 0; kd < 3; ++kd) {                                             \
            const char* q_ = wpb + ((long long)(((CC) * NPP + (P)) * 3 + kd)) * 2048;    \
            pwh[BUFI][kd] = *reinterpret_cast<const bf16x8*>(q_ + l16);                                \
            pwl[BUFI][kd] = *reinterpret_cast<const bf16x8*>(q_ + l16 + 1024u);                        \
        }
#define MVSGI_PL_READX(BUFI, P)                                                                        \
        {                                                                                              \
            const int t0_ = 2 * (P), t1_ = 2 * (P) + 1 < 9 ? 2 * (P) + 1 : 2 * (P);                    \
            const int o0_ = ((t0_ / 3) * ITW + t0_ % 3) * kVSB, o1_ = ((t1_ / 3) * ITW + t1_ % 3) * kVSB; \
            const int off_ = pbase + (second ? o1_ : o0_);                                             \
            _Pragma("unroll") for (int ip = 0; ip < PD; ++ip) {                                        \
                pxh[BUFI][ip] = *reinterpret_cast<const bf16x8*>(img + off_ + ip * (ITH * ITW * kVSB)); \
                pxl[BUFI][ip] = *reinterpret_cast<const bf16x8*>(img + off_ + ip * (ITH * ITW * kVSB) + 32); \
            }                                                                                          \
        }
#define MVSGI_PL_MFMAS(WBUFI, BUFI)                                                                         \
        _Pragma("unroll") for (int tr = 0; tr < 3; ++tr)                                               \
            _Pragma("unroll") for (int kd = 0; kd < 3; ++kd)                                           \
                _Pragma("unroll") for (int i = 0; i < TD; ++i)                                         \
                    acc[i][0] = mfma16<F16>(tr == 0 ? pwl[WBUFI][kd] : pwh[WBUFI][kd], tr == 1 ? pxl[BUFI][i + kd] : pxh[BUFI][i + kd], acc[i][0]);
        if constexpr (PLANE) {
            unsigned l16 = lane16;
            MVSGI_PL_LOADW(0, 0, 0)
            MVSGI_PL_LOADW(1, 0, 1)
        } else if constexpr (!WLDS) {
            unsigned l16 = lane16;
#pragma unroll
            for (int s0 = 0; s0 < LA; ++s0) { MVSGI_LOADWB(wpb + (DKU && od0 == 0 ? 9 * 2048 : 0), s0, 0, s0, ctc) }
        }
        STAMP()
        __syncthreads();
        STAMP()
        int k = 0, cc = 0;
        for (int u = 0; u < U; ++u) {
            const unsigned char* img = ldsb + (u & 1) * BUFW + (DKU && od0 == 0 ? ITH * ITW * kVSB : 0);
            const bool last = cc + 1 == nchunks;
            const bool more = u + 1 < U;
            const int ncc = last ? 0 : cc + 1;
            int ncb = cb_, nb = b_, nod0 = od0, noh0 = oh0, now0 = ow0;
            if (last && more) {
                MVSGI_DECODE((int)blockIdx.x + (k + 1) * G, ncb, nb, nod0, noh0, now0)
                MVSGI_CTILES(ctn, ncb)
            } else {
#pragma unroll
                for (int j = 0; j < NW; ++j) ctn[j] = ctc[j];
            }
            const char* const wpc_ = wpb + (DKU && od0 == 0 ? 9 * 2048 : 0);
            const char* const wpn_ = wpb + (DKU && nod0 == 0 ? 9 * 2048 : 0);
            f32x4 esc[NW], esh[NW], rres[RPRE ? MW : 1][RPRE ? NW : 1];
            int eoff[MW];
            int soff[MW];
            const int ypd = a.ys_2d ? 0 : 1, ypp = a.ys_2d ? 2 : 1;
#pragma unroll
            for (int j = 0; j < NW; ++j) {
                esc[j] = *reinterpret_cast<const f32x4*>(a.scale + ctc[j] * 16 + kg * 4);
                esh[j] = *reinterpret_cast<const f32x4*>(a.shift + ctc[j] * 16 + kg * 4);
            }
            if (last) {
#pragma unroll
                for (int i = 0; i < MW; ++i) {
                    const int od = od0 + tdv[i], oh = oh0 + thv[i], ow = ow0 + twv[i];
                    const bool inside = od < a.Do && oh < a.Ho && ow < a.Wo;
                    eoff[i] = inside ? ((od * a.Ho + oh) * a.Wo + ow) * a.Cout + kg * 4 : -1;
                    soff[i] = ((((od + ypd) * (a.Ho + 2 * ypp) + oh + ypp) * (a.Wo + 2 * ypp) + ow + ypp) * a.Cout) * 4 + (kg >> 1) * 16 + (kg & 1) * 8;
                }
            }
            if constexpr (PLANE) {
                MVSGI_PL_READX(0, 0)
#pragma unroll
                for (int p_ = 0; p_ < NPP + 1; ++p_) {
                    const int cur = p_ & 1, nxt = cur ^ 1;
                    unsigned l16 = lane16;
                    asm volatile("" : "+v"(l16));
                    if (p_ + 2 < NPP) {
                        MVSGI_PL_LOADW((p_ + 2) % 3, cc, p_ + 2)
                    } else if (p_ + 2 > NPP) {
                        MVSGI_PL_LOADW(p_ + 2 - (NPP + 1), ncc, p_ + 2 - (NPP + 1))
                    }
                    if (p_ < NPP) {
                        if (p_ + 1 < NPP) {
                            MVSGI_PL_READX(nxt, p_ + 1)
                        } else if (last && a.res) {
                            const float* rb = a.res + (long long)b_ * frame_elems;
#pragma unroll
                            for (int i = 0; i < MW; ++i)
                                rres[i][0] = *reinterpret_cast<const f32x4*>(rb + (eoff[i] >= 0 ? eoff[i] : 0));
                        }
                        MVSGI_PL_MFMAS(p_ % 3, cur)
                        if (p_ + 1 < NPP) {
#pragma unroll
                            for (int q_ = 0; q_ < 6 + 2 * PD; ++q_) {
                                __builtin_amdgcn_sched_group_barrier(0x008, 36 / (6 + 2 * PD) > 0 ? 36 / (6 + 2 * PD) : 1, 0);
                                __builtin_amdgcn_sched_group_barrier(0x120, 1, 0);
                            }
                            __builtin_amdgcn_sched_group_barrier(0x008, 36, 0);
                        }
                    }
                    __builtin_amdgcn_sched_barrier(0);
                }
            } else {
            if (XB >= 2) {
#pragma unroll
                for (int p0 = 0; p0 < XLA; ++p0) { MVSGI_READX(p0 % XB, p0, 0, MW) }
            } else {
                MVSGI_READX(0, 0, 0, MW)
            }
#pragma unroll
            for (int s_ = 0; s_ < NSLOT; ++s_) {
                const int wcur = s_ % WB;
                unsigned l16 = lane16;
                asm volatile("" : "+v"(l16));
                const int xcur = XB >= 2 ? (s_ % XB) : 0, xnxt = XB >= 2 ? ((s_ + XLA) % XB) : 0;
                if (!(MVSGI_ABL & 1) && !WLDS) {
                    if (s_ + LA < NSLOT) {
                        if (s_ + LA < kPairs) { MVSGI_LOADWB(wpc_, (s_ + LA) % WB, cc, s_ + LA, ctc) }
                    } else {
                        MVSGI_LOADWB(wpn_, (s_ + LA - NSLOT) % WB, ncc, s_ + LA - NSLOT, ctn)
                    }
                }
                if (RPRE && s_ == kPairs - 1 && last && a.res) {
                    const float* rb = a.res + (long long)b_ * frame_elems;
#pragma unroll
                    for (int i = 0; i < MW; ++i)
#pragma unroll
                        for (int j = 0; j < NW; ++j)
                            rres[i][j] = *reinterpret_cast<const f32x4*>(rb + (eoff[i] >= 0 ? eoff[i] + ctc[j] * 16 : 0));
                }
                if (s_ < kPairs - ((MVSGI_ABL & 32) ? 1 : 0)) {
                    if (XB >= 2) {
#define MVSGI_T0(SL) ((BRD != 0 && (SL) < 9) ? MW / 2 : 0)
#define MVSGI_T1(SL) (MW)
                        if (s_ + XLA < kPairs && !(MVSGI_ABL & 2)) MVSGI_READX(xnxt, s_ + XLA, MVSGI_T0(s_ + XLA), MVSGI_T1(s_ + XLA))
                        if (!(MVSGI_ABL & 16)) { MVSGI_MFMAS(wcur, xcur, MVSGI_T0(s_), MVSGI_T1(s_)) }
                        constexpr int NMEM = 2 * NW + 2 * MW, NMFMA = 3 * MW * NW;
                        constexpr int RATIO = NMFMA / NMEM > 0 ? NMFMA / NMEM : 1;
                        const bool full_ = MVSGI_T1(s_) - MVSGI_T0(s_) == MW && (s_ + XLA >= kPairs || MVSGI_T1(s_ + XLA) - MVSGI_T0(s_ + XLA) == MW);
                        if (full_) {
#pragma unroll
                        for (int q_ = 0; q_ < NMEM; ++q_) {
                            __builtin_amdgcn_sched_group_barrier(0x008, RATIO, 0);
                            __builtin_amdgcn_sched_group_barrier(0x120, 1, 0);
                        }
                        __builtin_amdgcn_sched_group_barrier(0x008, NMFMA, 0);
                        }
                    } else {
                        __builtin_amdgcn_sched_barrier(0);
                        MVSGI_MFMAS(wcur, 0, 0, MH)
                        __builtin_amdgcn_sched_barrier(0);
                        if (s_ + 1 < kPairs) MVSGI_READX(0, s_ + 1, 0, MH)
                        __builtin_amdgcn_sched_barrier(0);
                        MVSGI_MFMAS(wcur, 0, MH, MW)
                        __builtin_amdgcn_sched_barrier(0);
                        if (s_ + 1 < kPairs) MVSGI_READX(0, s_ + 1, MH, MW)
                    }
                }
                __builtin_amdgcn_sched_barrier(0);
            }
            }
            STAMP()
            if (last) {
                const int ct0 = (cb_ * WN + wn) * NW;
                float* yb = a.y + (long long)b_ * frame_elems;
                f32x4 rl[RPRE ? 1 : MW][RPRE ? 1 : NW];
                if (!RPRE && a.res) {
                    const float* rb = a.res + (long long)b_ * frame_elems;
#pragma unroll
                    for (int i = 0; i < (RPRE ? 1 : MW); ++i)
#pragma unroll
                        for (int j = 0; j < (RPRE ? 1 : NW); ++j)
                            rl[i][j] = *reinterpret_cast<const f32x4*>(rb + (eoff[i] >= 0 ? eoff[i] + ctc[j] * 16 : 0));
                }
#pragma unroll
                for (int i = 0; i < MW; ++i) {
#pragma unroll
                    for (int j = 0; j < NW; ++j) {
                        if (TACC) acc[i][j] = (acc[i][j] + acc1[i][j]) + acc2[i][j];
                        f32x4 r = acc[i][j] * esc[j] + esh[j];
                        if (a.res) r += RPRE ? rres[RPRE ? i : 0][RPRE ? j : 0] : rl[RPRE ? 0 : i][RPRE ? 0 : j];
#pragma unroll
                        for (int e = 0; e < 4; ++e) r[e] = r[e] > 0.f ? r[e] : r[e] * a.neg_slope;
                        if (a.y_split) {
                            u32x2 hi, lo;
                            split_x4<F16>(r, hi, lo, satm);
                            if (eoff[i] >= 0 && ct0 + j < CT) {
                                unsigned char* q = a.y_split + (long long)b_ * ((long long)(a.Do + 2 * ypd) * (a.Ho + 2 * ypp) * (a.Wo + 2 * ypp) * a.Cout * 4) +
                                                   soff[i] + (ct0 + j) * 64;
                                *reinterpret_cast<u32x2*>(q) = hi;
                                *reinterpret_cast<u32x2*>(q + 32) = lo;
                            }
                        } else if (eoff[i] >= 0 && ct0 + j < CT) *reinterpret_cast<f32x4*>(yb + eoff[i] + (ct0 + j) * 16) = r;
                        acc[i][j] = f32x4{0.f, 0.f, 0.f, 0.f};
                        if (TACC) acc1[i][j] = acc2[i][j] = f32x4{0.f, 0.f, 0.f, 0.f};
                    }
                }
                k += 1;
                cb_ = ncb; b_ = nb; od0 = nod0; oh0 = noh0; ow0 = now0;
#pragma unroll
                for (int j = 0; j < NW; ++j) ctc[j] = ctn[j];
            }
            cc = ncc;
            STAMP()
            __syncthreads();
            STAMP()
        }
#undef MVSGI_T0
#undef MVSGI_T1
#undef MVSGI_TAP
#undef MVSGI_PL_LOADW
#undef MVSGI_PL_READX
#undef MVSGI_PL_MFMAS
#undef MVSGI_CTILES
#undef MVSGI_LOADW
#undef MVSGI_READX
#undef MVSGI_MFMAS
    }
#undef MVSGI_DECODE
    STAMP()
#undef STAMP
    if constexpr (F16) sf_sat_report(a.sat, kSatSplit, satm, 65504.f);
}

template <int NW, int MW, int WM, int WN, int TD, int TH, int TW, int S, int KD = 3, bool UPS = false, bool PLANE = false,
          bool V32 = false, bool WLDS = false>
__global__ __launch_bounds__(512, 2) void conv3d_bf16x3_kernel(ConvArgs a) {
    conv3d_x3_body<NW, MW, WM, WN, TD, TH, TW, S, KD, UPS, PLANE, V32, WLDS, false>(a);
}
template <int NW, int MW, int WM, int WN, int TD, int TH, int TW, int S, int KD = 3, bool UPS = false, bool PLANE = false,
          bool V32 = false, bool WLDS = false>
__global__ __launch_bounds__(512, 2) void conv3d_f16x3_kernel(ConvArgs a) {
    conv3d_x3_body<NW, MW, WM, WN, TD, TH, TW, S, KD, UPS, PLANE, V32, WLDS, true>(a);
}

template <int NW, int MW, int WM, int WN, int TD, int TH, int TW>
__global__ __launch_bounds__(512, 2) void conv3d_bf16x3_d32_kernel(ConvArgs a) {
    conv3d_x3_body<NW, MW, WM, WN, TD, TH, TW, 1, 3, false, false, false, false, false, true>(a);
}
template <int NW, int MW, int WM, int WN, int TD, int TH, int TW>
__global__ __launch_bounds__(512, 2) void conv3d_f16x3_d32_kernel(ConvArgs a) {
    conv3d_x3_body<NW, MW, WM, WN, TD, TH, TW, 1, 3, false, false, false, false, true, true>(a);
}

template <int NW, int MW, int WM, int WN, int TD, int TH, int TW>
__global__ __launch_bounds__(512, 2) void conv3d_bf16x3_d32_dk_kernel(ConvArgs a) {
    conv3d_x3_body<NW, MW, WM, WN, TD, TH, TW, 1, 3, false, false, false, false, false, true, TD>(a);
}
template <int NW, int MW, int WM, int WN, int TD, int TH, int TW>
__global__ __launch_bounds__(512, 2) void conv3d_f16x3_d32_dk_kernel(ConvArgs a) {
    conv3d_x3_body<NW, MW, WM, WN, TD, TH, TW, 1, 3, false, false, false, false, true, true, TD>(a);
}
template <int NW, int MW, int WM, int WN, int TD, int TH, int TW>
__global__ __launch_bounds__(512, 2) void conv3d_bf16x3_d32u_dk_kernel(ConvArgs a) {
    conv3d_x3_body<NW, MW, WM, WN, TD, TH, TW, 1, 3, true, false, false, false, false, true, TD>(a);
}
template <int NW, int MW, int WM, int WN, int TD, int TH, int TW>
__global__ __launch_bounds__(512, 2) void conv3d_f16x3_d32u_dk_kernel(ConvArgs a) {
    conv3d_x3_body<NW, MW, WM, WN, TD, TH, TW, 1, 3, true, false, false, false, true, true, TD>(a);
}

template <int NW, int MW, int WM, int WN, int TD, int TH, int TW>
__global__ __launch_bounds__(512, 2) void conv3d_bf16x3_d32_dk2_kernel(ConvArgs a) {
    conv3d_x3_body<NW, MW, WM, WN, TD, TH, TW, 1, 3, false, false, false, false, false, true, 2>(a);
}
template <int NW, int MW, int WM, int WN, int TD, int TH, int TW>
__global__ __launch_bounds__(512, 2) void conv3d_f16x3_d32_dk2_kernel(ConvArgs a) {
    conv3d_x3_body<NW, MW, WM, WN, TD, TH, TW, 1, 3, false, false, false, false, true, true, 2>(a);
}

template <int NW, int MW, int WM, int WN, int TD, int TH, int TW, int BRD>
__global__ __launch_bounds__(512, 2) void conv3d_bf16x3_d32_brd_kernel(ConvArgs a) {
    conv3d_x3_body<NW, MW, WM, WN, TD, TH, TW, 1, 3, false, false, false, false, false, true, 3, BRD>(a);
}
template <int NW, int MW, int WM, int WN, int TD, int TH, int TW, int BRD>
__global__ __launch_bounds__(512, 2) void conv3d_f16x3_d32_brd_kernel(ConvArgs a) {
    conv3d_x3_body<NW, MW, WM, WN, TD, TH, TW, 1, 3, false, false, false, false, true, true, 3, BRD>(a);
}
template <int NW, int MW, int WM, int WN, int TD, int TH, int TW, int BRD>
__global__ __launch_bounds__(512, 2) void conv3d_bf16x3_d32u_brd_kernel(ConvArgs a) {
    conv3d_x3_body<NW, MW, WM, WN, TD, TH, TW, 1, 3, true, false, false, false, false, true, 3, BRD>(a);
}
template <int NW, int MW, int WM, int WN, int TD, int TH, int TW, int BRD>
__global__ __launch_bounds__(512, 2) void conv3d_f16x3_d32u_brd_kernel(ConvArgs a) {
    conv3d_x3_body<NW, MW, WM, WN, TD, TH, TW, 1, 3, true, false, false, false, true, true, 3, BRD>(a);
}

template <int NW, int MW, int WM, int WN, int TD, int TH, int TW>
__global__ __launch_bounds__(512, 2) void conv3d_bf16x3_d32u_kernel(ConvArgs a) {
    conv3d_x3_body<NW, MW, WM, WN, TD, TH, TW, 1, 3, true, false, false, false, false, true>(a);
}
template <int NW, int MW, int WM, int WN, int TD, int TH, int TW>
__global__ __launch_bounds__(512, 2) void conv3d_f16x3_d32u_kernel(ConvArgs a) {
    conv3d_x3_body<NW, MW, WM, WN, TD, TH, TW, 1, 3, true, false, false, false, true, true>(a);
}

template <int NW, int MW, int WM, int WN, int TD, int TH, int TW, int S, int KD = 3, bool UPS = false, bool PLANE = false,
          bool V32 = false, bool WLDS = false, bool F16 = false, bool D32 = false, bool DSK = false, int BRD = 0>
int launch_bf16x3(ConvArgs a, hipStream_t st) {
    constexpr int ITD = (TD - 1) * (KD == 1 ? 1 : S) + KD, ITH = (TH - 1) * S + 3, ITW = (TW - 1) * S + 3;
    constexpr int ROWP = V32 ? ((ITW * kVSB + 255) / 256) * 256 : ITW * kVSB;
    constexpr bool WARM = MVSGI_WARM && KD == 3 && !UPS && !PLANE && !V32 && !WLDS && S == 1 && MW * NW <= 2;
    static_assert(!D32 || (S == 1 && KD == 3 && !PLANE && !V32 && !WLDS), "32-channel slices: stride-1 3x3x3 variants");
    constexpr size_t lds_bytes = (size_t)2 * ((D32 ? 2 : 1) * ITD * ITH * ROWP + (WLDS ? NW * pairs_of(KD) * 2048 : 0)) + (WARM ? 4096 : 0);
    static_assert(lds_bytes <= 160 * 1024, "LDS images too large");
    void (*kern)(ConvArgs);
    static_assert(!DSK || (D32 && TD <= 2), "depth skip: 32-channel slices, one- or two-plane bricks");
    constexpr bool DKU = DSK && BRD == 3;
    static_assert(!DKU || (TD == 1 && !UPS), "per-unit depth skip: one-plane bricks");
    MVSGI_REQUIRE(!DSK || a.Do == (DKU ? 2 : TD), "conv3d: the depth-skip kernels serve volumes exactly %d planes deep (got %d)", DKU ? 2 : TD, a.Do);
    if constexpr (DKU && F16) kern = conv3d_f16x3_d32_dk2_kernel<NW, MW, WM, WN, TD, TH, TW>;
    else if constexpr (DKU) kern = conv3d_bf16x3_d32_dk2_kernel<NW, MW, WM, WN, TD, TH, TW>;
    else if constexpr (BRD != 0 && UPS && F16) kern = conv3d_f16x3_d32u_brd_kernel<NW, MW, WM, WN, TD, TH, TW, BRD>;
    else if constexpr (BRD != 0 && UPS) kern = conv3d_bf16x3_d32u_brd_kernel<NW, MW, WM, WN, TD, TH, TW, BRD>;
    else if constexpr (BRD != 0 && F16) kern = conv3d_f16x3_d32_brd_kernel<NW, MW, WM, WN, TD, TH, TW, BRD>;
    else if constexpr (BRD != 0) kern = conv3d_bf16x3_d32_brd_kernel<NW, MW, WM, WN, TD, TH, TW, BRD>;
    else if constexpr (DSK && UPS && F16) kern = conv3d_f16x3_d32u_dk_kernel<NW, MW, WM, WN, TD, TH, TW>;
    else if constexpr (DSK && UPS) kern = conv3d_bf16x3_d32u_dk_kernel<NW, MW, WM, WN, TD, TH, TW>;
    else if constexpr (DSK && F16) kern = conv3d_f16x3_d32_dk_kernel<NW, MW, WM, WN, TD, TH, TW>;
    else if constexpr (DSK) kern = conv3d_bf16x3_d32_dk_kernel<NW, MW, WM, WN, TD, TH, TW>;
    else if constexpr (D32 && UPS && F16) kern = conv3d_f16x3_d32u_kernel<NW, MW, WM, WN, TD, TH, TW>;
    else if constexpr (D32 && UPS) kern = conv3d_bf16x3_d32u_kernel<NW, MW, WM, WN, TD, TH, TW>;
    else if constexpr (D32 && F16) kern = conv3d_f16x3_d32_kernel<NW, MW, WM, WN, TD, TH, TW>;
    else if constexpr (D32) kern = conv3d_bf16x3_d32_kernel<NW, MW, WM, WN, TD, TH, TW>;
    else if constexpr (F16) kern = conv3d_f16x3_kernel<NW, MW, WM, WN, TD, TH, TW, S, KD, UPS, PLANE, V32, WLDS>;
    else kern = conv3d_bf16x3_kernel<NW, MW, WM, WN, TD, TH, TW, S, KD, UPS, PLANE, V32, WLDS>;
    MVSGI_REQUIRE(!D32 || a.Cin % 32 == 0, "conv3d: the 32-channel-slice kernels need Cin %% 32 == 0 (got %d)", a.Cin);
    static mvsgi::PersistentGeom geo_cache[mvsgi::kMaxDevices] = {};
    mvsgi::PersistentGeom geo;
    if (mvsgi::persistent_geometry(kern, 512, lds_bytes, 2, geo_cache, "conv3d(bf16x3)", geo)) return 1;
    a.tiles_h = (int)mvsgi::cdiv(a.Ho, TH);
    a.tiles_w = (int)mvsgi::cdiv(a.Wo, TW);
    const int CT = a.Cout / (V32 ? 32 : 16);
    constexpr bool kBorderSplit = D32 && !DSK && BRD == 0 && TD == 2 && WM == 2 && MW == 4 && TH == 4 && TW == 16 && S == 1;
    if constexpr (kBorderSplit) {
        const long long layer = (long long)a.B * a.tiles_h * a.tiles_w * mvsgi::cdiv(CT, WN * NW);
        if (a.od_cnt == 0 && a.Do == 4 && layer >= 4ll * geo.cus) {
            ConvArgs b = a;
            b.od_cnt = 1;
            b.od_off = 0;
            if (launch_bf16x3<NW, MW, WM, WN, TD, TH, TW, S, KD, UPS, PLANE, V32, WLDS, F16, D32, DSK, 1>(b, st)) return 1;
            b.od_off = 2;
            return launch_bf16x3<NW, MW, WM, WN, TD, TH, TW, S, KD, UPS, PLANE, V32, WLDS, F16, D32, DSK, 2>(b, st);
        }
    }
    a.tiles_d = a.od_cnt > 0 ? a.od_cnt : (int)mvsgi::cdiv(a.Do, TD);
    const long long nb = (long long)a.B * a.tiles_d * a.tiles_h * a.tiles_w * mvsgi::cdiv(CT, WN * NW);
    MVSGI_REQUIRE(nb < (1ll << 31), "conv3d: too many units");
    MVSGI_REQUIRE((long long)a.Din * a.Hin * a.Win * a.Cin < (1ll << 29), "conv3d: volume too large for 32-bit byte offsets");
    MVSGI_REQUIRE(!UPS || (a.Din % 2 == 0 && a.Hin % 2 == 0 && a.Win % 2 == 0), "conv3d: fused upsample needs even sizes");
    MVSGI_REQUIRE(!UPS || (long long)(a.Hin / 2) * (a.Win / 2) * a.Cin < (1ll << 23), "conv3d: fused upsample: low-resolution plane too large for 24-bit strides");
    MVSGI_REQUIRE((long long)a.Do * a.Ho * a.Wo * a.Cout < (1ll << 31), "conv3d: output frame too large for 32-bit element offsets");
    MVSGI_REQUIRE(!a.y_split || (!V32 && (long long)(a.Do + 2) * (a.Ho + 4) * (a.Wo + 4) * a.Cout * 4 < (1ll << 31)),
                  "conv3d: split-padded output not available for this kernel / size");
    a.total_units = (int)nb;
    MVSGI_SAT_WORDS(sat_words_);
    a.sat = sat_words_;
#ifdef MVSGI_STAMPS
    {
        static unsigned long long* dbgbuf = nullptr;
        const char* e_ = getenv("MVSGI_STAMP");
        if (e_ && !dbgbuf) { (void)hipMalloc(&dbgbuf, 8 * 128 * 8); (void)hipMemset(dbgbuf, 0, 8 * 128 * 8); }
        a.dbg = dbgbuf;
        if (e_ && atoi(e_) == 2 && dbgbuf) {
            static unsigned long long h[8 * 128];
            (void)hipDeviceSynchronize();
            (void)hipMemcpy(h, dbgbuf, sizeof(h), hipMemcpyDeviceToHost);
            for (int w = 0; w < 8; ++w) {
                fprintf(stderr, "wave %d:", w);
                for (int i = 0; i < 120; ++i) fprintf(stderr, " %lld", (long long)(h[w * 128 + i] - h[0]));
                fprintf(stderr, "\n");
            }
        }
    }
#endif
    hipLaunchKernelGGL(kern, dim3(mvsgi::persistent_grid(geo, nb)), dim3(512), lds_bytes, st, a);
    return mvsgi::check_launch("mvsgi_conv3d_f32(bf16x3)");
}
```

### mvs_gi_amd/csrc/conv3d_f16.hip

```cpp
#include "common.hpp"
#include "conv_common.hpp"
#include "conv3d_variants.hpp"
#ifdef MVSGI_STAMPS
#include <cstdio>
#include <cstdlib>
#endif

namespace {
#include "conv3d_bf16x3.hpp"
}

namespace mvsgi {

int conv3d_launch_b3_f16(int variant, const void* args, hipStream_t st) {
    const ConvArgs& a = *static_cast<const ConvArgs*>(args);
    switch (variant) {
#define MVSGI_MFMA(V, ...)
#define MVSGI_B3(V, K, ...) case V: return MVSGI_B3_LAUNCH##K(true, __VA_ARGS__)(a, st);
#include "conv3d_variants.inc"
#undef MVSGI_MFMA
#undef MVSGI_B3
    }
    return fail("mvsgi_conv3d_f32: variant %d has no fp16-split form (MVSGI_CONV_F16 goes with MVSGI_CONV_BF16X3 / _C16 / _V32)", variant);
}

}
```

### mvs_gi_amd/csrc/conv3d_variants.hpp

```cpp
#pragma once
namespace {
enum Variant {
    V_DIRECT1, V_DIRECT4, V_HEAD,
#define MVSGI_MFMA(V, ...) V,
#define MVSGI_B3(V, K, ...) V,
#include "conv3d_variants.inc"
#undef MVSGI_MFMA
#undef MVSGI_B3
    V_COUNT
};
}

#define MVSGI_B3_LAUNCH_kernel(F16, ...) launch_bf16x3<__VA_ARGS__, F16>
#define MVSGI_B3_LAUNCH_d32_kernel(F16, ...) launch_bf16x3<__VA_ARGS__, 1, 3, false, false, false, false, F16, true>
#define MVSGI_B3_LAUNCH_d32_dk_kernel(F16, ...) launch_bf16x3<__VA_ARGS__, 1, 3, false, false, false, false, F16, true, true>
#define MVSGI_B3_LAUNCH_d32_dk2_kernel(F16, ...) launch_bf16x3<__VA_ARGS__, 1, 3, false, false, false, false, F16, true, true, 3>
#define MVSGI_B3_LAUNCH_d32u_kernel(F16, ...) launch_bf16x3<__VA_ARGS__, 1, 3, true, false, false, false, F16, true>
#define MVSGI_B3_LAUNCH_d32u_dk_kernel(F16, ...) launch_bf16x3<__VA_ARGS__, 1, 3, true, false, false, false, F16, true, true>

namespace mvsgi {
int conv3d_launch_b3_f16(int variant, const void* args, hipStream_t st);
}
```

### mvs_gi_amd/dropin/common_modules.py

```python
from __future__ import annotations

import os

import copy
from typing import Dict, NamedTuple, Optional, Type

import torch
from torch import nn, Tensor

from .. import hip_ops as H


def module_getstate(self):
    return {k: v for k, v in self.__dict__.items() if not k.startswith("_mvsgi_")}


def _owned_split_buffer(owner, attr: str, key: tuple, make):
    bufs = owner.__dict__.setdefault(attr, {})
    if key not in bufs:
        bufs[key] = make()
    return bufs[key]


def _owned_head_buffer(self, B, D, Hh, W, C, device):
    bufs = self.__dict__.setdefault("_mvsgi_head_bufs", {})
    key = (D, Hh, W, C, device)
    ent = bufs.get(key)
    if ent is None or ent[0].B < B:
        big = H.SplitAct(B, D, Hh, W, C, device)
        keep = ent[1] + [ent[0]] if ent is not None and (ent[2] or ent[1]) else []
        ent = bufs[key] = [big, keep, False]
    if torch.cuda.is_current_stream_capturing():
        ent[2] = True
    big = ent[0]
    if big.B == B:
        return big
    return H.SplitAct(B, D, Hh, W, C, device, buf=big.buf[:B])


class NoOp(nn.Identity):
    def infer_size(self, in_size):
        return in_size


RELU_TYPE: Dict[str, Type[nn.Module]] = {"original": nn.ReLU, "leaky": nn.LeakyReLU, "none": NoOp}
NORM2D_TYPE: Dict[str, Type[nn.Module]] = {"batch": nn.BatchNorm2d, "instance": nn.InstanceNorm2d, "none": NoOp}
NORM3D_TYPE: Dict[str, Type[nn.Module]] = {"batch": nn.BatchNorm3d, "instance": nn.InstanceNorm3d, "none": NoOp}


_USE_D32 = os.environ.get("MVSGI_D32", "1") != "0"
_D32_OK: Dict[tuple, bool] = {}


class Packed(NamedTuple):
    wp: Tensor
    scale: object
    shift: object
    unscale: float = 1.0


class ConvLaunch:
    __slots__ = ("w", "wp", "scale", "shift", "stride", "neg_slope", "cin", "cout", "key", "inorm", "_cache")

    def __init__(self, w: Tensor, scale: Tensor, shift: Tensor, stride: int, neg_slope: float, inorm=None, key=None):
        self.w = w
        self.wp = H.pack_conv_weights(w)
        self.scale, self.shift = scale.contiguous(), shift.contiguous()
        self.stride, self.neg_slope, self.inorm, self.key = int(stride), neg_slope, inorm, key
        self.cout, self.cin = int(w.shape[0]), int(w.shape[1])
        self._cache: Dict[tuple, Packed] = {}

    def _cached(self, key: tuple, make) -> Packed:
        ent = self._cache.get(key)
        if ent is None:
            ent = self._cache[key] = make()
        return ent

    def _entry(self, packed) -> Packed:
        wp, unscale = packed if isinstance(packed, tuple) else (packed, None)
        return Packed(wp, self.scale if unscale is None else (self.scale * unscale).contiguous(), self.shift)

    def run(self, x_ndhwc: Tensor, res: Optional[Tensor] = None, impl: Optional[int] = None) -> Tensor:
        if self.inorm is not None:
            return self.inorm.apply(self._run_conv(x_ndhwc, None, impl), res)
        return self._run_conv(x_ndhwc, res, impl)

    def _run_conv(self, x_ndhwc: Tensor, res: Optional[Tensor] = None, impl: Optional[int] = None) -> Tensor:
        wp, scale = self.wp, self.scale
        if impl is None:
            impl = H.CONV_AUTO
            if H.split_mode() and self.cin % 16 == 0 and self.cout % 16 == 0:
                impl, wp, scale = self._stream(self._stream_layout(x_ndhwc.shape[:4]), H.mode_fmt())
        elif impl == H.CONV_BF16X3:
            wp = self._stream_packed(H.CONV_BF16X3, "bf16").wp
        return H.conv3d(x_ndhwc, self.w, wp, scale, self.shift, res=res, stride=self.stride, neg_slope=self.neg_slope, impl=impl)

    def _stream_layout(self, dims=None, up2: bool = False) -> int:
        if self._c16():
            return H.CONV_BF16X3_C16
        if dims is not None and _USE_D32 and H.split_mode() and self.cin % 32 == 0 and (up2 or (self.stride == 1 and self.cout % 16 == 0)):
            key = (up2, self.cin, self.cout) + tuple(dims)
            ok = _D32_OK.get(key)
            if ok is None:
                ok = _D32_OK[key] = H.conv3d_up2_d32_applies(dims[0], self.cin, *dims[1:], self.cout) if up2 else \
                    H.conv3d_d32_applies(dims[0], self.cin, *dims[1:], self.cout, self.stride)
            if ok:
                return H.CONV_BF16X3_D32
        return H.CONV_BF16X3

    def _stream_packed(self, layout: int, fmt: str) -> Packed:
        return self._cached(("stream", layout, fmt), lambda: self._entry(H._pack_conv3d_split(self.w, layout, fmt)))

    def _stream(self, layout: int, fmt: str):
        p = self._stream_packed(layout, fmt)
        return layout | (H.CONV_F16 if fmt == "f16" else 0), p.wp, p.scale

    def _c16(self) -> bool:
        return self.cout == 16 and self.stride == 1 and self.cin % 16 == 0

    def rs_ok(self) -> bool:
        return self.inorm is None and H.conv3d_rs_applies(self.cin, self.cout, self.stride, self.neg_slope)

    def _rs(self, fmt: str) -> Packed:
        return self._cached(("rs", fmt), lambda: self._entry(H.pack_conv_weights_rs(self.w, fmt)))

    def wino_ok(self, D: int, Hh: int, W: int) -> bool:
        return self.inorm is None and H.conv3d_wino_applies(self.cin, self.cout, D, Hh, W, self.stride, self.neg_slope)

    def _wino(self) -> Packed:
        return self._cached(("wino",), lambda: self._entry(H.pack_conv_weights_wino(self.w)))

    def s2rs_ok(self) -> bool:
        return self.inorm is None and H.split_mode() and H.conv3d_s2rs_applies(self.cin, self.cout, self.stride, self.neg_slope)

    def _s2(self, fmt: str) -> Packed:
        def make():
            if fmt == "bf16":
                return Packed(H.pack_conv_weights_s2rs(self.w, self.scale), None, self.shift)
            wp, up, un = H.pack_conv_weights_s2rs(self.w, self.scale, "f16")
            return Packed(wp, None, (self.shift * up).contiguous(), un)
        return self._cached(("s2", fmt), make)

    def poly_ok(self) -> bool:
        return self.inorm is None and H.split_mode() and self.stride == 1 and H.conv3d_up2_poly_applies(self.cin, self.cout, self.neg_slope)

    def _poly_plan(self, x_split) -> Packed:
        D, Hh, W, fmt = x_split.D, x_split.H, x_split.W, x_split.fmt
        return self._cached(("poly", D, Hh, W, fmt), lambda: self._entry(H.conv3d_up2_poly_plan(self.w, D, Hh, W, fmt=fmt)))

    def head_split_ok(self) -> bool:
        return self.inorm is None and H.split_mode() and self.cout == 1 and self.cin % 16 == 0 and self.stride == 1

    def run_head_split(self, x_split) -> Tensor:
        def make():
            if x_split.fmt == "f16":
                wp, unscale = H.pack_head_split_weights_f16(self.w)
                return Packed(wp, float(self.scale[0]) * unscale, float(self.shift[0]))
            return Packed(H.pack_head_split_weights(self.w), float(self.scale[0]), float(self.shift[0]))
        p = self._cached(("head", x_split.fmt), make)
        return H.conv3d_head_split(x_split, p.wp, p.scale, p.shift, neg_slope=self.neg_slope, f16=x_split.fmt == "f16")

    def run_up2_poly_split(self, x_split, out) -> "H.SplitAct":
        p = self._poly_plan(x_split)
        return H.conv3d_up2_poly_split(x_split, p.wp, p.scale, self.shift, out=out, neg_slope=self.neg_slope)

    def run_up2_poly(self, x_split, out=None) -> Tensor:
        p = self._poly_plan(x_split)
        return H.conv3d_up2_poly(x_split, p.wp, p.scale, self.shift, neg_slope=self.neg_slope, out=out)

    def run_up2_split(self, x_lowres_ndhwc: Tensor, res: Optional[Tensor], out) -> "H.SplitAct":
        _no_inorm(self, "run_up2_split")
        w_layout, wp, scale = self._stream(self._stream_layout(), H.mode_fmt())
        return H.conv3d_up2_out_split(x_lowres_ndhwc, wp, scale, self.shift, out=out, res=res, neg_slope=self.neg_slope, w_layout=w_layout)

    def can_fuse_up2(self) -> bool:
        return H.split_mode() and self.stride == 1 and self.cin % 16 == 0 and self.cout % 16 == 0

    def run_up2(self, x_lowres_ndhwc: Tensor, res: Optional[Tensor] = None) -> Tensor:
        if self.inorm is not None:
            return self.inorm.apply(self._run_up2(x_lowres_ndhwc, None), res)
        return self._run_up2(x_lowres_ndhwc, res)

    def _run_up2(self, x_lowres_ndhwc: Tensor, res: Optional[Tensor] = None) -> Tensor:
        w_layout, wp, scale = self._stream(self._stream_layout(x_lowres_ndhwc.shape[:4], up2=True), H.mode_fmt())
        return H.conv3d_up2(x_lowres_ndhwc, wp, scale, self.shift, res=res, neg_slope=self.neg_slope, w_layout=w_layout)


def _is_identity(m) -> bool:
    return m is None or isinstance(m, nn.Identity)


def _fingerprint(blk) -> tuple:
    conv = blk.conv_layer
    parts = [conv.weight.data_ptr(), conv.weight._version, tuple(conv.stride)]
    if conv.bias is not None:
        parts += [conv.bias.data_ptr(), conv.bias._version]
    parts += norm_key(blk.norm_layer)
    act = blk.activation
    parts += [type(act).__name__, float(getattr(act, "negative_slope", 0.0))]
    return tuple(parts)


_BN = (nn.BatchNorm3d, nn.BatchNorm2d)
_IN = (nn.InstanceNorm3d, nn.InstanceNorm2d)


def norm_key(norm) -> list:
    parts = [type(norm).__name__]
    if isinstance(norm, _BN + _IN):
        parts += [bool(norm.training), float(norm.eps), bool(getattr(norm, "track_running_stats", True))]
        for t in (norm.weight, norm.bias, norm.running_mean, norm.running_var):
            parts += [None, None] if t is None else [t.data_ptr(), t._version]
    return parts


class InstanceNormLaunch:
    __slots__ = ("gamma", "beta", "eps", "neg_slope")

    def apply(self, y: Tensor, res: Optional[Tensor] = None) -> Tensor:
        return H.instance_norm(y, res=res, gamma=self.gamma, beta=self.beta, eps=self.eps, neg_slope=self.neg_slope, out=y)


def _no_inorm(L, what: str) -> None:
    if L.inorm is not None:
        raise RuntimeError(f"{what}: this layer has an instance norm (its epilogue does not fold); use the plain fp32 path")


def lower_norm(norm, conv_bias: Optional[Tensor], cout: int, device, slope: float, dims: int = 3):
    bias = conv_bias.detach().float() if conv_bias is not None else None
    name = type(norm).__name__
    use_running = isinstance(norm, _BN) or (isinstance(norm, _IN) and norm.track_running_stats)
    if use_running:
        if norm.training:
            raise RuntimeError(f"HIP path implements eval-mode {name} only: call model.eval()")
        if norm.running_mean is None or norm.running_var is None:
            raise NotImplementedError(f"{name} without running statistics")
        gamma = norm.weight.detach().float() if norm.weight is not None else torch.ones(cout, device=device)
        beta = norm.bias.detach().float() if norm.bias is not None else torch.zeros(cout, device=device)
        alpha = gamma / torch.sqrt(norm.running_var.detach().float() + norm.eps)
        scale = alpha
        shift = beta - norm.running_mean.detach().float() * alpha
        if bias is not None:
            shift = shift + bias * alpha
        return scale, shift, None
    scale = torch.ones(cout, device=device, dtype=torch.float32)
    shift = bias.clone() if bias is not None else torch.zeros(cout, device=device, dtype=torch.float32)
    if _is_identity(norm):
        return scale, shift, None
    if isinstance(norm, _IN):
        if norm.affine and norm.num_features != cout:
            raise ValueError(f"{name}({norm.num_features}) after a conv with {cout} output channels")
        rec = InstanceNormLaunch()
        rec.gamma = norm.weight.detach().float().contiguous() if norm.affine and norm.weight is not None else None
        rec.beta = norm.bias.detach().float().contiguous() if norm.affine and norm.bias is not None else None
        rec.eps, rec.neg_slope = float(norm.eps), float(slope)
        return scale, shift, rec
    raise NotImplementedError(f"norm layer {name} has no HIP implementation "
                              f"(only BatchNorm{dims}d in eval mode, InstanceNorm{dims}d and NoOp)")


def act_slope(act) -> float:
    if isinstance(act, nn.LeakyReLU):
        return float(act.negative_slope)
    if isinstance(act, nn.ReLU):
        return 0.0
    if _is_identity(act):
        return 1.0
# ... 111 lines not shown
```

### mvs_gi_amd/dropin/polyphase.py

```python
from __future__ import annotations

from typing import Dict, Tuple

import numpy as np

FIRST, INT, LAST, ONLY = 0, 1, 2, 3
CLASS_NAMES = ("first", "int", "last", "only")


def cell_class(i: int, n: int) -> int:
    if n == 1:
        return ONLY
    return FIRST if i == 0 else (LAST if i == n - 1 else INT)


def class_cell(cls: int, n: int) -> int:
    return {FIRST: 0, INT: 1, LAST: n - 1, ONLY: 0}[cls]


def axis_matrix(p: int, i: int, n: int) -> np.ndarray:
    M = np.zeros((3, 3))
    for k in range(3):
        v = 2 * i + p + k - 1
        if v < 0 or v >= 2 * n:
            continue
        m, q = divmod(v, 2)
        taps = ((m - 1, 0.25), (m, 0.75)) if q == 0 else ((m, 0.75), (m + 1, 0.25))
        for src, wgt in taps:
            src = min(max(src, 0), n - 1)
            M[src - i + 1][k] += wgt
    return M


def class_matrix(p: int, cls: int) -> np.ndarray:
    n = {FIRST: 4, INT: 4, LAST: 4, ONLY: 1}[cls]
    return axis_matrix(p, class_cell(cls, n), n)


def effective_weights(w: np.ndarray, Md: np.ndarray, Mh: np.ndarray, Mw: np.ndarray) -> np.ndarray:
    return np.einsum("ak,bl,cm,oiklm->oiabc", Md, Mh, Mw, np.asarray(w, np.float64), optimize=True)


def main_weight_sets(w: np.ndarray) -> Dict[Tuple[int, int, int], np.ndarray]:
    co = w.shape[0]
    out = {}
    for pd in range(2):
        for cd in (FIRST, INT, LAST, ONLY):
            for ph in range(2):
                parts = [effective_weights(w, class_matrix(pd, cd), class_matrix(ph, INT), class_matrix(pw, INT)) for pw in range(2)]
                out[(pd, cd, ph)] = np.concatenate(parts, axis=0).astype(np.float32).reshape(2 * co, w.shape[1], 3, 3, 3)
    return out


def face_delta(p: int, cls: int) -> np.ndarray:
    d = class_matrix(p, cls) - class_matrix(p, INT)
    if cls != INT:
        if cls in (FIRST, ONLY):
            d[0] = 0.0
        if cls in (LAST, ONLY):
            d[2] = 0.0
    return d
```

### mvs_gi_amd/hip_ops.py

```python
from __future__ import annotations

from typing import Optional

import torch

from . import _lib

import ctypes
import math
import os

CONV_AUTO, CONV_DIRECT, CONV_MFMA, CONV_BF16X3, CONV_BF16X3_C16, CONV_BF16X3_V32, CONV_BF16X3_D32 = 0, 1, 2, 3, 4, 5, 6
SPLIT_F16 = 1
CONV_F16 = 0x100

CONV_MODES = ("f32", "bf16x3", "f16x3")
_CONV_MODE = os.environ.get("MVSGI_CONV_MODE", "f16x3")
if _CONV_MODE not in CONV_MODES:
    raise ValueError(f"MVSGI_CONV_MODE={_CONV_MODE!r} not in {CONV_MODES}")




def set_conv_mode(mode: str) -> None:
    global _CONV_MODE
    if mode not in CONV_MODES:
        raise ValueError(f"conv mode {mode!r} not in {CONV_MODES}")
    _CONV_MODE = mode


def get_conv_mode() -> str:
    return _CONV_MODE


SAT_SWEEP, SAT_SPLIT, SAT_WINO = 1, 2, 4
_SAT_TEXT = {SAT_SWEEP: "the sweep's cost volume reached +-65504 (un-normalised features?)",
             SAT_SPLIT: "an activation written or staged in fp16 pieces reached +-65504",
             SAT_WINO: "an activation of the Winograd-form level reached its +-16376 range (or a transformed sum +-65504)"}
RANGE_CHECKS = ("raise", "warn", "off")
_RANGE_CHECK = os.environ.get("MVSGI_RANGE_CHECK", "raise")
if _RANGE_CHECK not in RANGE_CHECKS:
    raise ValueError(f"MVSGI_RANGE_CHECK={_RANGE_CHECK!r} not in {RANGE_CHECKS}")
_RANGE_WARNED = set()
_RANGE_SEEN = 0


class MvsgiRangeError(RuntimeError):
    """The fp16 split left its range: results since the last check are saturated, not the reference's."""


def set_range_check(policy: str) -> None:
    global _RANGE_CHECK
    if policy not in RANGE_CHECKS:
        raise ValueError(f"range check policy {policy!r} not in {RANGE_CHECKS}")
    _RANGE_CHECK = policy


def get_range_check() -> str:
    return _RANGE_CHECK


def saturation_flags(clear: bool = False) -> int:
    import ctypes
    out = ctypes.c_uint(0)
    if _lib.load().mvsgi_saturation_flags(1 if clear else 0, ctypes.byref(out)) != 0:
        return 0
    return int(out.value)


def saturation_words():
    import ctypes
    out = (ctypes.c_uint * 8)()
    if _lib.load().mvsgi_saturation_words(out) != 0:
        return [0] * 8
    return [int(v) for v in out]


def range_flags_seen() -> int:
    return _RANGE_SEEN


def check_range(where: str = "", sync_device=None) -> int:
    if _RANGE_CHECK == "off":
        return 0
    if sync_device is not None:
        torch.cuda.synchronize(sync_device)
    f = saturation_flags(clear=False)
    if not f:
        return 0
    words = saturation_words()
    saturation_flags(clear=True)
    global _RANGE_SEEN
    _RANGE_SEEN |= f
    what = "; ".join(t for b, t in _SAT_TEXT.items() if f & b)
    msg = (f"mvs_gi_amd{' (' + where + ')' if where else ''}: the fp16 split (MVSGI_CONV_MODE=f16x3, the default) left its range (flags 0x{f:x}, words {words[:4]}) -- {what}. "
# ... 191 lines not shown
        return sweep_std_valid(feats, grids, sweep_validity(grids, grid_masks, masks))
    B, N, C, Hi, Wi = feats.shape
    f = _feats_nhwc(feats) if nhwc else _dev(feats, "feats")
    grids, gm, gm_f32, masks, (D, Ho, Wo, Hm, Wm) = _rig_args(grids, grid_masks, masks, B, N)
    vol = torch.empty((B, D, Ho, Wo, C), device=f.device, dtype=torch.float32)
    _call("mvsgi_sweep_std_nhwc_f32" if nhwc else "mvsgi_sweep_std_f32", f.data_ptr(), grids.data_ptr(), gm.data_ptr(), gm_f32,
          masks.data_ptr(), vol.data_ptr(), B, N, C, Hi, Wi, Hm, Wm, D, Ho, Wo, _stream_ptr(f))
    return vol


def sweep_cat(feats, grids, layout: str = "auto") -> torch.Tensor:
    nhwc = layout == "auto" and feats.dim() == 5 and feats.shape[2] % 4 == 0
    f = _feats_nhwc(feats) if nhwc else _dev(feats, "feats")
    B, N, C, Hi, Wi = feats.shape
    grids = _dev(grids, "grids")
    Bg, Ng, D, Ho, Wo, two = grids.shape
    if (Bg, Ng, two) != (B, N, 2):
        raise AssertionError(f"grids {tuple(grids.shape)} do not match feats {tuple(feats.shape)}")
    vol = torch.empty((B, D, Ho, Wo, N * C), device=f.device, dtype=torch.float32)
    _call("mvsgi_sweep_cat_nhwc_f32" if nhwc else "mvsgi_sweep_cat_f32", f.data_ptr(), grids.data_ptr(), vol.data_ptr(), B, N, C, Hi, Wi,
          D, Ho, Wo, _stream_ptr(f))
    return vol


def pack_conv_weights(w_oidhw: torch.Tensor) -> Optional[torch.Tensor]:
    lib = _lib.load()
    w = _dev(w_oidhw, "conv weight")
    Cout, Cin = w.shape[:2]
    if tuple(w.shape[2:]) != (3, 3, 3):
        raise NotImplementedError(f"only 3x3x3 kernels are supported, got {tuple(w.shape[2:])}")
    if Cin % 16 or not (Cout % 16 == 0 or Cout == 1):
        return None
    wp = torch.empty(lib.mvsgi_conv3d_packed_weight_floats(Cout, Cin), device=w.device, dtype=torch.float32)
    _call("mvsgi_conv3d_pack_weights_f32", w.data_ptr(), wp.data_ptr(), Cout, Cin, _stream_ptr(w))
    return wp


def _pack_conv3d_split(w_oidhw: torch.Tensor, layout: int, fmt: str = "bf16"):
    lib = _lib.load()
    w = _dev(w_oidhw, "conv weight")
    Cout, Cin = w.shape[:2]
    if tuple(w.shape[2:]) != (3, 3, 3) or Cin % 16 or Cout % 16 or (layout == CONV_BF16X3_C16 and Cout != 16) or \
            (layout == CONV_BF16X3_V32 and Cout % 32) or (layout == CONV_BF16X3_D32 and Cin % 32):
        return None
    unscale = None
    if fmt == "f16":
        up, unscale = _pow2_unscale(w.abs().amax(dim=(1, 2, 3, 4)))
        w = (w * up.view(-1, 1, 1, 1, 1)).contiguous()
    n = {CONV_BF16X3: lambda: lib.mvsgi_conv3d_packed_weight_bytes_bf16x3(Cout, Cin),
         CONV_BF16X3_C16: lambda: lib.mvsgi_conv3d_packed_weight_bytes_bf16x3_c16(Cin),
         CONV_BF16X3_D32: lambda: lib.mvsgi_conv3d_packed_weight_bytes_bf16x3(Cout, Cin),
         CONV_BF16X3_V32: lambda: lib.mvsgi_conv3d_packed_weight_bytes_bf16x3_v32(Cout, Cin)}[layout]()
    wp = torch.empty(n, device=w.device, dtype=torch.uint8)
    _call("mvsgi_conv3d_pack_weights_split", w.data_ptr(), wp.data_ptr(), Cout, Cin, layout | (CONV_F16 if _fmt_code(fmt) else 0),
          _stream_ptr(w))
    return wp, (None if unscale is None else unscale.contiguous())


def _pack_bf16(w_oidhw: torch.Tensor, layout: int) -> Optional[torch.Tensor]:
    p = _pack_conv3d_split(w_oidhw, layout)
    return None if p is None else p[0]


def pack_conv_weights_bf16x3(w_oidhw: torch.Tensor) -> Optional[torch.Tensor]:
    return _pack_bf16(w_oidhw, CONV_BF16X3)


def pack_conv_weights_f16x3(w_oidhw: torch.Tensor, layout: int = CONV_BF16X3):
    return _pack_conv3d_split(w_oidhw, layout, "f16")


def pack_conv_weights_bf16x3_d32(w_oidhw: torch.Tensor) -> Optional[torch.Tensor]:
    return _pack_bf16(w_oidhw, CONV_BF16X3_D32)


def pack_conv_weights_bf16x3_v32(w_oidhw: torch.Tensor) -> Optional[torch.Tensor]:
    return _pack_bf16(w_oidhw, CONV_BF16X3_V32)


def pack_conv_weights_bf16x3_c16(w_oidhw: torch.Tensor) -> Optional[torch.Tensor]:
    return _pack_bf16(w_oidhw, CONV_BF16X3_C16)


def conv3d_d32_applies(B, Cin, Din, Hin, Win, Cout, stride=1) -> bool:
    return bool(_lib.load().mvsgi_conv3d_d32_applies(B, Cin, Din, Hin, Win, Cout, stride))


def conv3d_up2_d32_applies(B, Cin, Dl, Hl, Wl, Cout) -> bool:
    return bool(_lib.load().mvsgi_conv3d_up2_d32_applies(B, Cin, Dl, Hl, Wl, Cout))


def conv3d_v32_applies(B, Cin, Din, Hin, Win, Cout, stride=1) -> bool:
    return bool(_lib.load().mvsgi_conv3d_v32_applies(B, Cin, Din, Hin, Win, Cout, stride))


def _split_layout_bytes(layout: int, Cout: int, Cin: int) -> int:
    lib = _lib.load()
    layout &= ~CONV_F16
    if layout == CONV_BF16X3_C16:
        return lib.mvsgi_conv3d_packed_weight_bytes_bf16x3_c16(Cin)
    if layout == CONV_BF16X3_V32:
        return lib.mvsgi_conv3d_packed_weight_bytes_bf16x3_v32(Cout, Cin)
    if layout in (CONV_BF16X3, CONV_BF16X3_D32):
        return lib.mvsgi_conv3d_packed_weight_bytes_bf16x3(Cout, Cin)
    raise ValueError(f"w_layout {layout} is not one of the streaming split kernel's layouts")


def _conv3d_packed(w_packed, name: str, device, impl: int, Cout: int, Cin: int) -> Optional[int]:
    base = impl & ~CONV_F16
    split = base in (CONV_BF16X3_C16, CONV_BF16X3_V32, CONV_BF16X3_D32) or (base == CONV_BF16X3 and Cin % 16 == 0 and Cout % 16 == 0)
    if w_packed is None:
        if split:
            raise AssertionError(f"{name}: impl {impl} needs the packed weights of its layout")
        return None
    if split:
        return _arg(w_packed, name, device, torch.uint8, nbytes=_split_layout_bytes(base, Cout, Cin)).data_ptr()
    if base == CONV_DIRECT:
        return _arg(w_packed, name, device, _PACKED).data_ptr()
    packs = Cin % 16 == 0 and (Cout % 16 == 0 or Cout == 1)
    return _arg(w_packed, name, device, numel=_lib.load().mvsgi_conv3d_packed_weight_floats(Cout, Cin) if packs else None).data_ptr()


def conv3d(x, w_oidhw, w_packed, scale, shift, res=None, stride=1, neg_slope=0.01, impl=CONV_AUTO, out=None):
    x = _dev(x, "x")
    B, Din, Hin, Win, Cin = x.shape
    dev = x.device
    sc, sh, Cout = _scale_shift(scale, shift, dev)
    Do, Ho, Wo = (Din - 1) // stride + 1, (Hin - 1) // stride + 1, (Win - 1) // stride + 1
    shp = (B, Do, Ho, Wo, Cout)
    y = torch.empty(shp, device=dev, dtype=torch.float32) if out is None else _arg(out, "out", dev, shape=shp)
    _call("mvsgi_conv3d_f32", x.data_ptr(), _opt(w_oidhw, "w_oidhw", dev, shape=(Cout, Cin, 3, 3, 3)),
          _conv3d_packed(w_packed, "w_packed", dev, impl, Cout, Cin), sc, sh, _opt(res, "res", dev, shape=shp), y.data_ptr(), B, Cin, Din,
          Hin, Win, Cout, stride, float(neg_slope), impl, _stream_ptr(x))
    return y


def conv3d_up2(x, w_packed_b3, scale, shift, res=None, neg_slope=0.01, out=None, w_layout=CONV_BF16X3):
    x = _dev(x, "x")
    B, Dl, Hl, Wl, Cin = x.shape
    dev = x.device
    sc, sh, Cout = _scale_shift(scale, shift, dev)
    shp = (B, 2 * Dl, 2 * Hl, 2 * Wl, Cout)
    wp = _arg(w_packed_b3, "w_packed_b3", dev, torch.uint8, nbytes=_split_layout_bytes(w_layout, Cout, Cin))
    y = torch.empty(shp, device=dev, dtype=torch.float32) if out is None else _arg(out, "out", dev, shape=shp)
    _call("mvsgi_conv3d_up2_f32", x.data_ptr(), wp.data_ptr(), w_layout, sc, sh, _opt(res, "res", dev, shape=shp), y.data_ptr(), B, Cin, Dl,
          Hl, Wl, Cout, float(neg_slope), _stream_ptr(x))
    return y


def conv3d_up2_out_split(x, w_packed_b3, scale, shift, out: "SplitAct", res=None, neg_slope=0.01, w_layout=CONV_BF16X3) -> "SplitAct":
    x = _dev(x, "x")
    B, Dl, Hl, Wl, Cin = x.shape
    dev = x.device
    sc, sh, Cout = _scale_shift(scale, shift, dev)
    shp = (B, 2 * Dl, 2 * Hl, 2 * Wl, Cout)
    yp = _split_ptr(out, "out", dev, shp)
    wp = _arg(w_packed_b3, "w_packed_b3", dev, torch.uint8, nbytes=_split_layout_bytes(w_layout, Cout, Cin))
    _call("mvsgi_conv3d_up2_f32_out_split", x.data_ptr(), wp.data_ptr(), w_layout, sc, sh, _opt(res, "res", dev, shape=shp),
          yp, B, Cin, Dl, Hl, Wl, Cout, float(neg_slope), _stream_ptr(x))
    out.fmt = "f16" if w_layout & CONV_F16 else "bf16"
    return out


def conv3d_up2_poly_applies(cin: int, cout: int, neg_slope: float) -> bool:
    return cin == 32 and cout == 16 and 0.0 <= neg_slope <= 1.0


def conv3d_up2_poly_plan(w_oidhw: torch.Tensor, D: int, H: int, W: int, fmt: str = "bf16"):
    lib = _lib.load()
    if tuple(w_oidhw.shape) != (16, 32, 3, 3, 3):
        raise AssertionError(f"polyphase plan needs a [16, 32, 3, 3, 3] weight, got {tuple(w_oidhw.shape)}")
    n = lib.mvsgi_conv3d_up2_poly_plan_bytes(D, H, W)
    if not n:
        raise RuntimeError("mvsgi_conv3d_up2_poly_plan_bytes: bad dims")
    wh = w_oidhw.detach().to("cpu", torch.float32).contiguous()
    unscale = None
    if fmt == "f16":
        up, un = _pow2_unscale(wh.abs().amax(dim=(1, 2, 3, 4)))
        wh = (wh * up.view(-1, 1, 1, 1, 1)).contiguous()
        unscale = un.to(w_oidhw.device)
    plan = torch.empty(n, dtype=torch.uint8)
    _call("mvsgi_conv3d_up2_poly_plan_fmt", wh.data_ptr(), plan.data_ptr(), D, H, W, _fmt_code(fmt))
    plan = plan.to(w_oidhw.device)
    return (plan, unscale) if fmt == "f16" else plan


def _poly_plan_ptr(plan, device, x: "SplitAct") -> int:
# ... 1419 lines not shown
```

Before: 6309.

## Fold depth upsampling into conv weights for fused up2 conv3d

```diff
diff --git a/include/mvsgi.h b/include/mvsgi.h
--- a/include/mvsgi.h
+++ b/include/mvsgi.h
@@ -19,6 +19,10 @@
 #define MVSGI_CONV_BF16X3_C16 4
 #define MVSGI_CONV_BF16X3_V32 5
 #define MVSGI_CONV_BF16X3_D32 6
+
+#define MVSGI_CONV_BF16X3_UPF 7
+
+#define MVSGI_CONV_BF16X3_UPF_D32 8
 
 #define MVSGI_CONV_F16 0x100
 
@@ -82,6 +86,8 @@
 int mvsgi_conv3d_v32_applies(int B, int Cin, int Din, int Hin, int Win, int Cout, int stride);
 int mvsgi_conv3d_d32_applies(int B, int Cin, int Din, int Hin, int Win, int Cout, int stride);
 int mvsgi_conv3d_up2_d32_applies(int B, int Cin, int Dl, int Hl, int Wl, int Cout);
+int mvsgi_conv3d_up2_upf_applies(int B, int Cin, int Dl, int Hl, int Wl, int Cout);
+size_t mvsgi_conv3d_packed_weight_bytes_upf(int Cout, int Cin);
 size_t mvsgi_conv3d_packed_weight_bytes_bf16x3_v32(int Cout, int Cin);
 int mvsgi_conv3d_pack_weights_bf16x3_v32(const float* w_oidhw, void* w_packed, int Cout, int Cin, mvsgi_stream_t stream);
 size_t mvsgi_conv3d_packed_weight_bytes_bf16x3_c16(int Cin);
diff --git a/mvs_gi_amd/_lib.py b/mvs_gi_amd/_lib.py
--- a/mvs_gi_amd/_lib.py
+++ b/mvs_gi_amd/_lib.py
@@ -41,6 +41,8 @@
     "mvsgi_conv3d_v32_applies": (c_int, [c_int] * 7),
     "mvsgi_conv3d_d32_applies": (c_int, [c_int] * 7),
     "mvsgi_conv3d_up2_d32_applies": (c_int, [c_int] * 6),
+    "mvsgi_conv3d_up2_upf_applies": (c_int, [c_int] * 6),
+    "mvsgi_conv3d_packed_weight_bytes_upf": (c_size_t, [c_int, c_int]),
     "mvsgi_conv3d_packed_weight_bytes_bf16x3_v32": (c_size_t, [c_int, c_int]),
     "mvsgi_conv3d_pack_weights_bf16x3_v32": (c_int, [_P, _P, c_int, c_int, _P]),
     "mvsgi_conv3d_packed_weight_bytes_bf16x3_c16": (c_size_t, [c_int]),
diff --git a/mvs_gi_amd/csrc/conv3d.hip b/mvs_gi_amd/csrc/conv3d.hip
--- a/mvs_gi_amd/csrc/conv3d.hip
+++ b/mvs_gi_amd/csrc/conv3d.hip
@@ -245,7 +245,26 @@
     return a.Cout == 32 ? big >= 384 : mid * mvsgi::cdiv(a.Cout, 64) >= 384;
 }
 
+int select_variant_up2(const ConvArgs& a, int w_layout);
+
+int upf_variant(const ConvArgs& a, bool pays) {
+    if (a.Cin % 16 || a.Cout != 32 || a.Do < 4 || a.Do % 2) return V_COUNT;
+    if (!pays) return B3UF_N32;
+    ConvArgs b = a;
+    static const float dummy = 0.f;
+    if (!b.wp) b.wp = reinterpret_cast<const f32x4*>(&dummy);
+    const long long big = (long long)a.B * mvsgi::cdiv(a.Do, 4) * mvsgi::cdiv(a.Ho, 4) * mvsgi::cdiv(a.Wo, 16);
+    return big >= 384 && select_variant_up2(b, MVSGI_CONV_BF16X3) == B3U_N32 ? B3UF_N32 : V_COUNT;
+}
+
 int select_variant_up2(const ConvArgs& a, int w_layout) {
+    if (w_layout == MVSGI_CONV_BF16X3_UPF || w_layout == MVSGI_CONV_BF16X3_UPF_D32) {
+        int v = upf_variant(a, false);
+        if (v != V_COUNT && w_layout == MVSGI_CONV_BF16X3_UPF_D32) v = a.Cin % 32 ? V_COUNT : B3UFD_N32;
+        if (v == V_COUNT) mvsgi::fail("mvsgi_conv3d_up2_f32: the depth-folded kernels do not apply to this problem (see mvsgi_conv3d_up2_upf_applies)");
+        else if (!a.wp) { mvsgi::fail("mvsgi_conv3d_up2_f32: needs w_packed (depth-folded layout)"); return V_COUNT; }
+        return v;
+    }
     if (w_layout == MVSGI_CONV_BF16X3_D32) {
         const int base = a.Cin % 32 ? V_COUNT : select_variant_up2(a, MVSGI_CONV_BF16X3);
         const bool d2 = a.Do == 2;
@@ -424,6 +443,7 @@
 #define MVSGI_MFMA(V, ...) case V: return launch_mfma<__VA_ARGS__>(a, st);
 #define MVSGI_B3(V, K, ...) case V: return MVSGI_B3_LAUNCH##K(false, __VA_ARGS__)(a, st);
 #include "conv3d_variants.inc"
+#include "conv3d_upf_variants.inc"
 #undef MVSGI_MFMA
 #undef MVSGI_B3
     }
@@ -473,6 +493,7 @@
 #define MVSGI_MFMA(V, ...) case V: return "conv3d_mfma_kernel<" #__VA_ARGS__ ">";
 #define MVSGI_B3(V, K, ...) case V: return a.f16 ? "conv3d_f16x3" #K "<" #__VA_ARGS__ ">" : "conv3d_bf16x3" #K "<" #__VA_ARGS__ ">";
 #include "conv3d_variants.inc"
+#include "conv3d_upf_variants.inc"
 #undef MVSGI_MFMA
 #undef MVSGI_B3
     }
@@ -530,6 +551,16 @@
                       "mvsgi_conv3d_pack_weights_split: clearing the unused tail of the 32-channel-slice layout failed");
         hipLaunchKernelGGL(pack_weights_bf16x3_d32_kernel, dim3((unsigned)mvsgi::cdiv(total, 256)), dim3(256), 0, mvsgi::as_stream(stream),
                            w_oidhw, wp, Cout, Cin, f16);
+    } else if (layout == MVSGI_CONV_BF16X3_UPF || layout == MVSGI_CONV_BF16X3_UPF_D32) {
+        const bool d32 = layout == MVSGI_CONV_BF16X3_UPF_D32;
+        MVSGI_REQUIRE(!d32 || Cin % 32 == 0, "mvsgi_conv3d_pack_weights_split: the 32-channel-slice layout needs Cin %% 32 == 0 (got %d)", Cin);
+        const size_t set = mvsgi_conv3d_packed_weight_bytes_bf16x3(Cout, Cin);
+        for (int c = 0; c < 4; ++c) {
+            if (mvsgi_conv3d_pack_weights_split(w_oidhw + (size_t)c * Cout * Cin * 27, static_cast<char*>(w_packed) + c * set, Cout, Cin,
+                                                (d32 ? MVSGI_CONV_BF16X3_D32 : MVSGI_CONV_BF16X3) | (f16 ? MVSGI_CONV_F16 : 0), stream))
+                return 1;
+        }
+        return 0;
     } else {
         return mvsgi::fail("mvsgi_conv3d_pack_weights_split: layout %d is not a split-kernel layout", layout);
     }
@@ -648,7 +679,8 @@
     const bool f16 = (w_layout & MVSGI_CONV_F16) != 0;
     w_layout &= ~MVSGI_CONV_F16;
     MVSGI_REQUIRE(w_layout == MVSGI_CONV_BF16X3 || (w_layout == MVSGI_CONV_BF16X3_C16 && Cout == 16) ||
-                      (w_layout == MVSGI_CONV_BF16X3_V32 && Cout % 32 == 0) || (w_layout == MVSGI_CONV_BF16X3_D32 && Cin % 32 == 0),
+                      (w_layout == MVSGI_CONV_BF16X3_V32 && Cout % 32 == 0) || (w_layout == MVSGI_CONV_BF16X3_D32 && Cin % 32 == 0) ||
+                      w_layout == MVSGI_CONV_BF16X3_UPF || (w_layout == MVSGI_CONV_BF16X3_UPF_D32 && Cin % 32 == 0),
                   "mvsgi_conv3d_up2_f32: w_layout %d not valid for Cout %d", w_layout, Cout);
     MVSGI_REQUIRE(x && y && scale && shift && w_packed, "mvsgi_conv3d_up2_f32: null pointer");
     MVSGI_REQUIRE(Dl > 0 && Hl > 0 && Wl > 0 && Dl < (1 << 20) && Hl < (1 << 20) && Wl < (1 << 20),
@@ -668,7 +700,8 @@
                                               float neg_slope, mvsgi_stream_t stream) {
     const bool f16 = (w_layout & MVSGI_CONV_F16) != 0;
     w_layout &= ~MVSGI_CONV_F16;
-    MVSGI_REQUIRE(w_layout == MVSGI_CONV_BF16X3 || (w_layout == MVSGI_CONV_BF16X3_C16 && Cout == 16),
+    MVSGI_REQUIRE(w_layout == MVSGI_CONV_BF16X3 || (w_layout == MVSGI_CONV_BF16X3_C16 && Cout == 16) || w_layout == MVSGI_CONV_BF16X3_UPF ||
+                      (w_layout == MVSGI_CONV_BF16X3_UPF_D32 && Cin % 32 == 0),
                   "mvsgi_conv3d_up2_f32_out_split: w_layout %d not valid for Cout %d", w_layout, Cout);
     MVSGI_REQUIRE(x && y_split && scale && shift && w_packed, "mvsgi_conv3d_up2_f32_out_split: null pointer");
     MVSGI_REQUIRE(Dl > 0 && Hl > 0 && Wl > 0 && Dl < (1 << 20) && Hl < (1 << 20) && Wl < (1 << 20),
@@ -694,6 +727,17 @@
     return (base == B3U_N64 || base == B3U_N96) ? 1 : 0;
 }
 
+extern "C" int mvsgi_conv3d_up2_upf_applies(int B, int Cin, int Dl, int Hl, int Wl, int Cout) {
+    ConvArgs a{};
+    static const float dummy = 0.f;
+    if (Cin % 16 || Cout % 16 || Dl <= 0 || Hl <= 0 || Wl <= 0 ||
+        fill_args(a, &dummy, nullptr, &dummy, &dummy, &dummy, nullptr, nullptr, B, Cin, 2 * Dl, 2 * Hl, 2 * Wl, Cout, 1, 1.f))
+        return 0;
+    return upf_variant(a, true) != V_COUNT ? 1 : 0;
+}
+
+extern "C" size_t mvsgi_conv3d_packed_weight_bytes_upf(int Cout, int Cin) { return 4 * mvsgi_conv3d_packed_weight_bytes_bf16x3(Cout, Cin); }
+
 extern "C" const char* mvsgi_conv3d_up2_variant_f32(int B, int Cin, int Dl, int Hl, int Wl, int Cout, int w_layout) {
     ConvArgs a{};
     static const float dummy = 0.f;
diff --git a/mvs_gi_amd/csrc/conv3d_bf16x3.hpp b/mvs_gi_amd/csrc/conv3d_bf16x3.hpp
--- a/mvs_gi_amd/csrc/conv3d_bf16x3.hpp
+++ b/mvs_gi_amd/csrc/conv3d_bf16x3.hpp
@@ -187,7 +187,7 @@
     wp[o + 64] = __builtin_bit_cast(bf16x8, lo);
 }
 
-template <int NW, int MW, int WM, int WN, int TD, int TH, int TW, int S, int KD, bool UPS, bool PLANE, bool V32, bool WLDS, bool F16, bool D32 = false, int DK = 3, int BRD = 0>
+template <int NW, int MW, int WM, int WN, int TD, int TH, int TW, int S, int KD, bool UPS, bool PLANE, bool V32, bool WLDS, bool F16, bool D32 = false, int DK = 3, int BRD = 0, bool UPF = false>
 __device__ __forceinline__ void conv3d_x3_body(const ConvArgs& a) {
     static_assert(!WLDS || (WN == 1 && KD == 3 && !UPS && !PLANE && !V32 && S == 1 && NW == 1 && MW <= 2), "LDS-staged weights: one shared cout tile, one or two voxel tiles per wave");
     static_assert(!V32 || (S == 1 && KD == 3 && TW == 16 && TH % 2 == 0 && !PLANE), "32x32x16 schedule: stride 1, 16-wide even bricks");
@@ -195,6 +195,8 @@
                   "plane schedule: Cout == 16, 4 h-rows x TD planes x 16 w per brick");
     static_assert(!UPS || (S == 1 && KD == 3 && TD % 2 == 0 && TH % 2 == 0 && TW % 2 == 0),
                   "fused upsample: stride 1, even bricks (halo bricks are whole 2x2x2 cells)");
+    static_assert(!UPF || (UPS && DK == 3 && BRD == 0 && !PLANE && !V32 && WM == TD && MW * 16 == TH * TW),
+                  "depth fold: fused-upsample bricks whose waves own whole planes");
     static_assert(WM * WN == 4, "4 consumer waves per workgroup");
     static_assert(WM * MW * (V32 ? 32 : 16) == TD * TH * TW, "brick must be covered by the voxel tiles");
     static_assert(KD == 3 || (KD == 1 && TD == 1), "2-D bricks are one plane thick");
@@ -204,7 +206,7 @@
     constexpr bool DKU = D32 && TD == 1 && DK == 2;
     constexpr int kTaps = KD * 9, kPairs = D32 ? 9 * DK : pairs_of(KD);
     constexpr int kWBlk = D32 ? 27 : kPairs;
-    constexpr int ITD = (TD - 1) * SD + KD, ITH = (TH - 1) * S + 3, ITW = (TW - 1) * S + 3;
+    constexpr int ITD = UPF ? TD / 2 + 2 : (TD - 1) * SD + KD, ITH = (TH - 1) * S + 3, ITW = (TW - 1) * S + 3;
     constexpr int IV = ITD * ITH * ITW;
     constexpr int QB = D32 ? 3 : 2;
     constexpr int NIT = (IV * (1 << QB) + 255) / 256;
@@ -267,7 +269,136 @@
 
     if (producer) {
         const int ptid = tid - 256;
-        if constexpr (UPS) {
+        if constexpr (UPS && UPF) {
+            constexpr int CH = ITH / 2, CW = ITW / 2, NC = ITD * CH * CW;
+            constexpr int NCQ = NC << QB;
+            constexpr int NITU = (NCQ + 255) / 256;
+            const int Dl = a.Din >> 1, Hl = a.Hin >> 1, Wl = a.Win >> 1;
+            const int sH_ = Wl * a.Cin, sD_ = Hl * sH_;
+            int lo_d[NITU], lo_h[NITU], lo_w[NITU];
+            unsigned inmask[NITU];
+            const float* xb = a.x;
+            f32x4 crA[NITU][4], crB[NITU][4];
+            unsigned imA[NITU], imB[NITU];
+#define MVSGI_PLAN_UPF(UNIT)                                                                            \
+            {                                                                                           \
+                int cb_, b_, od_, oh_, ow_;                                                             \
+                MVSGI_DECODE(UNIT, cb_, b_, od_, oh_, ow_)                                              \
+                (void)cb_;                                                                              \
+                _Pragma("unroll") for (int it = 0; it < NITU; ++it) {                                   \
+                    const int c = (ptid + it * 256) >> QB;                                              \
+                    const int cw = c % CW, ch = (c / CW) % CH, pd = c / (CW * CH);                      \
+                    const int gh = oh_ - 1 + 2 * ch, gw = ow_ - 1 + 2 * cw;                             \
+                    lo_d[it] = (od_ >> 1) - 1 + pd;                                                     \
+                    lo_h[it] = (gh - 1) >> 1;                                                           \
+                    lo_w[it] = (gw - 1) >> 1;                                                           \
+                    inmask[it] = (gh >= 0 && gh < a.Hin ? 1u : 0u) | (gh + 1 < a.Hin ? 2u : 0u) |       \
+                                 (gw >= 0 && gw < a.Win ? 4u : 0u) | (gw + 1 < a.Win ? 8u : 0u);        \
+                }                                                                                       \
+                xb = a.x + (long long)b_ * Dl * Hl * Wl * a.Cin;                                        \
+            }
+#define MVSGI_CLAMP(V, N) ((V) < 0 ? 0 : ((V) > (N) - 1 ? (N) - 1 : (V)))
+            int k2 = 0, cc2 = 0;
+#define MVSGI_ISSUE_UPF_BEGIN()                                                                         \
+            if (cc2 == 0 && k2 > 0) { MVSGI_PLAN_UPF((int)blockIdx.x + k2 * G) }
+#define MVSGI_ISSUE_UPF1(CR, IM, IT)                                                                    \
+            {                                                                                           \
+                const int q = (ptid + (IT) * 256) & ((1 << QB) - 1);                                    \
+                const bool live = ptid + (IT) * 256 < NCQ;                                              \
+                const int d0 = live ? MVSGI_CLAMP(lo_d[IT], Dl) : 0;                                    \
+                const int h0 = live ? MVSGI_CLAMP(lo_h[IT], Hl) : 0, h1 = live ? MVSGI_CLAMP(lo_h[IT] + 1, Hl) : 0; \
+                const int w0 = live ? MVSGI_CLAMP(lo_w[IT], Wl) : 0, w1 = live ? MVSGI_CLAMP(lo_w[IT] + 1, Wl) : 0; \
+                const int cofs = cc2 * (D32 ? 32 : 16) + q * 4;                                         \
+                const int od_ = __mul24(d0, sD_), oh_[2] = {__mul24(h0, sH_), __mul24(h1, sH_)};        \
+                const int ow_[2] = {__mul24(w0, a.Cin) + cofs, __mul24(w1, a.Cin) + cofs};              \
+                _Pragma("unroll") for (int k = 0; k < 4; ++k)                                           \
+                    CR[IT][k] = *reinterpret_cast<const f32x4*>(xb + (od_ + oh_[(k >> 1) & 1] + ow_[k & 1])); \
+                IM[IT] = inmask[IT];                                                                    \
+            }
+#define MVSGI_ISSUE_UPF_END()                                                                           \
+            {                                                                                           \
+                if (++cc2 == nchunks) { cc2 = 0; ++k2; }                                                \
+                if (k2 >= nmine) { k2 = nmine - 1; cc2 = nchunks - 1; }                                 \
+            }
+#define MVSGI_ISSUE_UPF(CR, IM)                                                                         \
+            {                                                                                           \
+                MVSGI_ISSUE_UPF_BEGIN()                                                                 \
+                _Pragma("unroll") for (int it = 0; it < NITU; ++it) MVSGI_ISSUE_UPF1(CR, IM, it)        \
+                MVSGI_ISSUE_UPF_END()                                                                   \
+            }
+#define MVSGI_LERP2(A, B, O0, O1)      \
+            {                                                                                           \
+                const f32x4 d_ = fma4((A), f32x4{-1.f, -1.f, -1.f, -1.f}, (B));                         \
+                O0 = fma4(d_, f32x4{0.25f, 0.25f, 0.25f, 0.25f}, (A));                                  \
+                O1 = fma4(d_, f32x4{0.75f, 0.75f, 0.75f, 0.75f}, (A));                                  \
+            }
+#define MVSGI_PUT_UPF1(CR, IM, DST, IT)                                                                 \
+            {                                                                                           \
+                const int e = ptid + (IT) * 256;                                                        \
+                if (e < NCQ) {                                                                          \
+                    const int c = e >> QB, q = e & 3, sub_ = D32 ? ((e >> 2) & 1) * SUB : 0;            \
+                    const int cw = c % CW, ch = (c / CW) % CH, pd = c / (CW * CH);                      \
+                     \
+                    f32x4 xw[2][2], xo[2][2];                                                           \
+                    _Pragma("unroll") for (int k = 0; k < 2; ++k)                                       \
+                        MVSGI_LERP2(CR[IT][2 * k], CR[IT][2 * k + 1], xw[k][0], xw[k][1])               \
+                    _Pragma("unroll") for (int kw = 0; kw < 2; ++kw)                                    \
+                        MVSGI_LERP2(xw[0][kw], xw[1][kw], xo[0][kw], xo[1][kw])                         \
+                    _Pragma("unroll") for (int kh = 0; kh < 2; ++kh)                                    \
+                        _Pragma("unroll") for (int kw = 0; kw < 2; ++kw) {                              \
+                            const bool ok = ((IM[IT] >> kh) & (IM[IT] >> (2 + kw)) & 1u) != 0;          \
+                            u32x2 hi, lo;                                                               \
+                            split_x4<F16>(xo[kh][kw], hi, lo, satm);                                    \
+                            if (!ok) hi = lo = u32x2{0u, 0u};                                           \
+                            const int vo_ = (pd * ITH + 2 * ch + kh) * ROWP + (2 * cw + kw) * kVSB;     \
+                            *reinterpret_cast<u32x2*>((DST) + sub_ + vo_ + q * 8) = hi;                 \
+                            *reinterpret_cast<u32x2*>((DST) + sub_ + vo_ + 32 + q * 8) = lo;            \
+                        }                                                                               \
+                }                                                                                       \
+            }
+#define MVSGI_PUT_UPF(CR, IM, DST)                                                                      \
+            { _Pragma("unroll") for (int it = 0; it < NITU; ++it) MVSGI_PUT_UPF1(CR, IM, DST, it) }
+#define MVSGI_STEP_UPF(NEW, IMNEW, OLD, IMOLD, DST, DOPUT)                                              \
+            {                                                                                           \
+                MVSGI_ISSUE_UPF_BEGIN()                                                                 \
+                _Pragma("unroll") for (int it = 0; it < NITU; ++it) {                                   \
+                    MVSGI_ISSUE_UPF1(NEW, IMNEW, it)                                                    \
+                    if (DOPUT) MVSGI_PUT_UPF1(OLD, IMOLD, DST, it)                                      \
+                    __builtin_amdgcn_sched_barrier(0);                                                  \
+                }                                                                                       \
+                MVSGI_ISSUE_UPF_END()                                                                   \
+            }
+            STAMP()
+            MVSGI_PLAN_UPF((int)blockIdx.x)
+            MVSGI_ISSUE_UPF(crA, imA)
+            MVSGI_PUT_UPF(crA, imA, ldsb)
+            MVSGI_ISSUE_UPF(crA, imA)
+            STAMP()
+            __syncthreads();
+            STAMP()
+            for (int u = 0; u < U; u += 2) {
+                MVSGI_STEP_UPF(crB, imB, crA, imA, ldsb + ((u + 1) & 1) * BUF, u + 1 < U)
+                STAMP()
+                __syncthreads();
+                STAMP()
+                if (u + 1 < U) {
+                    MVSGI_STEP_UPF(crA, imA, crB, imB, ldsb + ((u + 2) & 1) * BUF, u + 2 < U)
+                    STAMP()
+                    __syncthreads();
+                    STAMP()
+                }
+            }
+#undef MVSGI_ISSUE_UPF
+#undef MVSGI_PUT_UPF
+#undef MVSGI_LERP2
+#undef MVSGI_ISSUE_UPF_BEGIN
+#undef MVSGI_ISSUE_UPF1
+#undef MVSGI_ISSUE_UPF_END
+#undef MVSGI_PUT_UPF1
+#undef MVSGI_STEP_UPF
+#undef MVSGI_PLAN_UPF
+#undef MVSGI_CLAMP
+        } else if constexpr (UPS) {
             constexpr int CD = ITD / 2, CH = ITH / 2, CW = ITW / 2, NC = CD * CH * CW;
             constexpr int NCQ = NC << QB;
             constexpr int NITU = (NCQ + 255) / 256;
@@ -762,7 +893,7 @@
         for (int i = 0; i < MW; ++i) {
             const int v = (wm * MW + i) * 16 + col;
             const int w_ = v % TW, h_ = BSK ? 2 * wm + (i & 1) : (v / TW) % TH, d_ = BSK ? (BRD == 2 ? 1 - (i >> 1) : (i >> 1)) : v / (TW * TH);
-            base[i] = (((d_ * SD) * ITH + h_ * S) * ITW + w_ * S) * kVSB + (kg >> 1) * 16;
+            base[i] = ((((UPF ? d_ >> 1 : d_) * SD) * ITH + h_ * S) * ITW + w_ * S) * kVSB + (kg >> 1) * 16;
         }
         int tdv[MW], thv[MW], twv[MW];
 #pragma unroll
@@ -780,6 +911,8 @@
         }
         const long long frame_elems = (long long)a.Do * a.Ho * a.Wo * a.Cout;
         int ctc[NW], ctn[NW];
+        const long long upf_set = UPF ? (long long)(a.Cin / 16) * CT * pairs_of(3) * 2048 : 0;
+#define MVSGI_UPF_W(OD0) (UPF ? upf_set * ((OD0) + wm == 0 ? 0 : (OD0) + wm == a.Do - 1 ? 3 : 1 + (((OD0) + wm) & 1)) : 0)
 #define MVSGI_CTILES(DST, CB)                                                         \
         _Pragma("unroll") for (int j = 0; j < NW; ++j) {                              \
             const int c_ = ((CB) * WN + wn) * NW + j;                                 \
@@ -874,7 +1007,7 @@
         } else if constexpr (!WLDS) {
             unsigned l16 = lane16;
 #pragma unroll
-            for (int s0 = 0; s0 < LA; ++s0) { MVSGI_LOADWB(wpb + (DKU && od0 == 0 ? 9 * 2048 : 0), s0, 0, s0, ctc) }
+            for (int s0 = 0; s0 < LA; ++s0) { MVSGI_LOADWB(wpb + (DKU && od0 == 0 ? 9 * 2048 : 0) + MVSGI_UPF_W(od0), s0, 0, s0, ctc) }
         }
         STAMP()
         __syncthreads();
@@ -893,8 +1026,8 @@
 #pragma unroll
                 for (int j = 0; j < NW; ++j) ctn[j] = ctc[j];
             }
-            const char* const wpc_ = wpb + (DKU && od0 == 0 ? 9 * 2048 : 0);
-            const char* const wpn_ = wpb + (DKU && nod0 == 0 ? 9 * 2048 : 0);
+            const char* const wpc_ = wpb + (DKU && od0 == 0 ? 9 * 2048 : 0) + MVSGI_UPF_W(od0);
+            const char* const wpn_ = wpb + (DKU && nod0 == 0 ? 9 * 2048 : 0) + MVSGI_UPF_W(nod0);
             f32x4 esc[NW], esh[NW], rres[RPRE ? MW : 1][RPRE ? NW : 1];
             int eoff[MW];
             int soff[MW];
@@ -1051,6 +1184,7 @@
             __syncthreads();
             STAMP()
         }
+#undef MVSGI_UPF_W
 #undef MVSGI_T0
 #undef MVSGI_T1
 #undef MVSGI_TAP
@@ -1140,10 +1274,28 @@
     conv3d_x3_body<NW, MW, WM, WN, TD, TH, TW, 1, 3, true, false, false, false, true, true>(a);
 }
 
+template <int NW, int MW, int WM, int WN, int TD, int TH, int TW>
+__global__ __launch_bounds__(512, 2) void conv3d_bf16x3_upf_kernel(ConvArgs a) {
+    conv3d_x3_body<NW, MW, WM, WN, TD, TH, TW, 1, 3, true, false, false, false, false, false, 3, 0, true>(a);
+}
+template <int NW, int MW, int WM, int WN, int TD, int TH, int TW>
+__global__ __launch_bounds__(512, 2) void conv3d_f16x3_upf_kernel(ConvArgs a) {
+    conv3d_x3_body<NW, MW, WM, WN, TD, TH, TW, 1, 3, true, false, false, false, true, false, 3, 0, true>(a);
+}
+
+template <int NW, int MW, int WM, int WN, int TD, int TH, int TW>
+__global__ __launch_bounds__(512, 2) void conv3d_bf16x3_upfd_kernel(ConvArgs a) {
+    conv3d_x3_body<NW, MW, WM, WN, TD, TH, TW, 1, 3, true, false, false, false, false, true, 3, 0, true>(a);
+}
+template <int NW, int MW, int WM, int WN, int TD, int TH, int TW>
+__global__ __launch_bounds__(512, 2) void conv3d_f16x3_upfd_kernel(ConvArgs a) {
+    conv3d_x3_body<NW, MW, WM, WN, TD, TH, TW, 1, 3, true, false, false, false, true, true, 3, 0, true>(a);
+}
+
 template <int NW, int MW, int WM, int WN, int TD, int TH, int TW, int S, int KD = 3, bool UPS = false, bool PLANE = false,
-          bool V32 = false, bool WLDS = false, bool F16 = false, bool D32 = false, bool DSK = false, int BRD = 0>
+          bool V32 = false, bool WLDS = false, bool F16 = false, bool D32 = false, bool DSK = false, int BRD = 0, bool UPF = false>
 int launch_bf16x3(ConvArgs a, hipStream_t st) {
-    constexpr int ITD = (TD - 1) * (KD == 1 ? 1 : S) + KD, ITH = (TH - 1) * S + 3, ITW = (TW - 1) * S + 3;
+    constexpr int ITD = UPF ? TD / 2 + 2 : (TD - 1) * (KD == 1 ? 1 : S) + KD, ITH = (TH - 1) * S + 3, ITW = (TW - 1) * S + 3;
     constexpr int ROWP = V32 ? ((ITW * kVSB + 255) / 256) * 256 : ITW * kVSB;
     constexpr bool WARM = MVSGI_WARM && KD == 3 && !UPS && !PLANE && !V32 && !WLDS && S == 1 && MW * NW <= 2;
     static_assert(!D32 || (S == 1 && KD == 3 && !PLANE && !V32 && !WLDS), "32-channel slices: stride-1 3x3x3 variants");
@@ -1154,7 +1306,13 @@
     constexpr bool DKU = DSK && BRD == 3;
     static_assert(!DKU || (TD == 1 && !UPS), "per-unit depth skip: one-plane bricks");
     MVSGI_REQUIRE(!DSK || a.Do == (DKU ? 2 : TD), "conv3d: the depth-skip kernels serve volumes exactly %d planes deep (got %d)", DKU ? 2 : TD, a.Do);
-    if constexpr (DKU && F16) kern = conv3d_f16x3_d32_dk2_kernel<NW, MW, WM, WN, TD, TH, TW>;
+    static_assert(!UPF || (UPS && !DSK && BRD == 0 && !PLANE && !V32 && !WLDS), "depth fold: a fused-upsample variant");
+    MVSGI_REQUIRE(!UPF || (a.Do >= 4 && a.Do % 2 == 0), "conv3d: the depth-folded fused upsample needs an even upsampled depth >= 4 (got %d)", a.Do);
+    if constexpr (UPF && D32 && F16) kern = conv3d_f16x3_upfd_kernel<NW, MW, WM, WN, TD, TH, TW>;
+    else if constexpr (UPF && D32) kern = conv3d_bf16x3_upfd_kernel<NW, MW, WM, WN, TD, TH, TW>;
+    else if constexpr (UPF && F16) kern = conv3d_f16x3_upf_kernel<NW, MW, WM, WN, TD, TH, TW>;
+    else if constexpr (UPF) kern = conv3d_bf16x3_upf_kernel<NW, MW, WM, WN, TD, TH, TW>;
+    else if constexpr (DKU && F16) kern = conv3d_f16x3_d32_dk2_kernel<NW, MW, WM, WN, TD, TH, TW>;
     else if constexpr (DKU) kern = conv3d_bf16x3_d32_dk2_kernel<NW, MW, WM, WN, TD, TH, TW>;
     else if constexpr (BRD != 0 && UPS && F16) kern = conv3d_f16x3_d32u_brd_kernel<NW, MW, WM, WN, TD, TH, TW, BRD>;
     else if constexpr (BRD != 0 && UPS) kern = conv3d_bf16x3_d32u_brd_kernel<NW, MW, WM, WN, TD, TH, TW, BRD>;
diff --git a/mvs_gi_amd/csrc/conv3d_f16.hip b/mvs_gi_amd/csrc/conv3d_f16.hip
--- a/mvs_gi_amd/csrc/conv3d_f16.hip
+++ b/mvs_gi_amd/csrc/conv3d_f16.hip
@@ -18,6 +18,7 @@
 #define MVSGI_MFMA(V, ...)
 #define MVSGI_B3(V, K, ...) case V: return MVSGI_B3_LAUNCH##K(true, __VA_ARGS__)(a, st);
 #include "conv3d_variants.inc"
+#include "conv3d_upf_variants.inc"
 #undef MVSGI_MFMA
 #undef MVSGI_B3
     }
diff --git a/mvs_gi_amd/csrc/conv3d_upf_variants.inc b/mvs_gi_amd/csrc/conv3d_upf_variants.inc
--- /dev/null
+++ b/mvs_gi_amd/csrc/conv3d_upf_variants.inc
@@ -0,0 +1,2 @@
+MVSGI_B3(B3UF_N32, _upf_kernel, 2, 4, 4, 1, 4, 4, 16)
+MVSGI_B3(B3UFD_N32, _upfd_kernel, 2, 4, 4, 1, 4, 4, 16)
diff --git a/mvs_gi_amd/csrc/conv3d_variants.hpp b/mvs_gi_amd/csrc/conv3d_variants.hpp
--- a/mvs_gi_amd/csrc/conv3d_variants.hpp
+++ b/mvs_gi_amd/csrc/conv3d_variants.hpp
@@ -5,6 +5,7 @@
 #define MVSGI_MFMA(V, ...) V,
 #define MVSGI_B3(V, K, ...) V,
 #include "conv3d_variants.inc"
+#include "conv3d_upf_variants.inc"
 #undef MVSGI_MFMA
 #undef MVSGI_B3
     V_COUNT
@@ -17,6 +18,8 @@
 #define MVSGI_B3_LAUNCH_d32_dk2_kernel(F16, ...) launch_bf16x3<__VA_ARGS__, 1, 3, false, false, false, false, F16, true, true, 3>
 #define MVSGI_B3_LAUNCH_d32u_kernel(F16, ...) launch_bf16x3<__VA_ARGS__, 1, 3, true, false, false, false, F16, true>
 #define MVSGI_B3_LAUNCH_d32u_dk_kernel(F16, ...) launch_bf16x3<__VA_ARGS__, 1, 3, true, false, false, false, F16, true, true>
+#define MVSGI_B3_LAUNCH_upf_kernel(F16, ...) launch_bf16x3<__VA_ARGS__, 1, 3, true, false, false, false, F16, false, false, 0, true>
+#define MVSGI_B3_LAUNCH_upfd_kernel(F16, ...) launch_bf16x3<__VA_ARGS__, 1, 3, true, false, false, false, F16, true, false, 0, true>
 
 namespace mvsgi {
 int conv3d_launch_b3_f16(int variant, const void* args, hipStream_t st);
diff --git a/mvs_gi_amd/dropin/common_modules.py b/mvs_gi_amd/dropin/common_modules.py
--- a/mvs_gi_amd/dropin/common_modules.py
+++ b/mvs_gi_amd/dropin/common_modules.py
@@ -50,6 +50,7 @@
 
 _USE_D32 = os.environ.get("MVSGI_D32", "1") != "0"
 _D32_OK: Dict[tuple, bool] = {}
+_USE_UPF = os.environ.get("MVSGI_UPF", "1") != "0"
 
 
 class Packed(NamedTuple):
@@ -108,7 +109,19 @@
                 return H.CONV_BF16X3_D32
         return H.CONV_BF16X3
 
+    def _up2_layout(self, dims, d32: bool) -> int:
+        if _USE_UPF and H.split_mode() and self.cout == 32 and self.cin % 16 == 0:
+            key = ("upf", self.cin, self.cout) + tuple(dims)
+            ok = _D32_OK.get(key)
+            if ok is None:
+                ok = _D32_OK[key] = H.conv3d_up2_upf_applies(dims[0], self.cin, *dims[1:], self.cout)
+            if ok:
+                return H.CONV_BF16X3_UPF_D32 if (_USE_D32 and self.cin % 32 == 0) else H.CONV_BF16X3_UPF
+        return self._stream_layout(dims, up2=True) if d32 else self._stream_layout()
+
     def _stream_packed(self, layout: int, fmt: str) -> Packed:
+        if layout in (H.CONV_BF16X3_UPF, H.CONV_BF16X3_UPF_D32):
+            return self._cached(("stream", layout, fmt), lambda: self._entry(H.pack_conv_weights_upf(self.w, fmt, layout)))
         return self._cached(("stream", layout, fmt), lambda: self._entry(H._pack_conv3d_split(self.w, layout, fmt)))
 
     def _stream(self, layout: int, fmt: str):
@@ -170,7 +183,7 @@
 
     def run_up2_split(self, x_lowres_ndhwc: Tensor, res: Optional[Tensor], out) -> "H.SplitAct":
         _no_inorm(self, "run_up2_split")
-        w_layout, wp, scale = self._stream(self._stream_layout(), H.mode_fmt())
+        w_layout, wp, scale = self._stream(self._up2_layout(x_lowres_ndhwc.shape[:4], d32=False), H.mode_fmt())
         return H.conv3d_up2_out_split(x_lowres_ndhwc, wp, scale, self.shift, out=out, res=res, neg_slope=self.neg_slope, w_layout=w_layout)
 
     def can_fuse_up2(self) -> bool:
@@ -182,7 +195,7 @@
         return self._run_up2(x_lowres_ndhwc, res)
 
     def _run_up2(self, x_lowres_ndhwc: Tensor, res: Optional[Tensor] = None) -> Tensor:
-        w_layout, wp, scale = self._stream(self._stream_layout(x_lowres_ndhwc.shape[:4], up2=True), H.mode_fmt())
+        w_layout, wp, scale = self._stream(self._up2_layout(x_lowres_ndhwc.shape[:4], d32=True), H.mode_fmt())
         return H.conv3d_up2(x_lowres_ndhwc, wp, scale, self.shift, res=res, neg_slope=self.neg_slope, w_layout=w_layout)
 
 
diff --git a/mvs_gi_amd/dropin/polyphase.py b/mvs_gi_amd/dropin/polyphase.py
--- a/mvs_gi_amd/dropin/polyphase.py
+++ b/mvs_gi_amd/dropin/polyphase.py
@@ -52,6 +52,27 @@
     return out
 
 
+D_FIRST, D_EVEN, D_ODD, D_LAST = 0, 1, 2, 3
+DEPTH_CLASS_NAMES = ("first", "even", "odd", "last")
+
+
+def depth_class(o: int, n_up: int) -> int:
+    return D_FIRST if o == 0 else (D_LAST if o == n_up - 1 else (D_ODD if o & 1 else D_EVEN))
+
+
+def depth_fold_matrices() -> np.ndarray:
+    F = np.zeros((4, 3, 3))
+    F[D_EVEN] = [[.75, .25, 0.], [.25, .75, .75], [0., 0., .25]]
+    F[D_ODD] = [[.25, 0., 0.], [.75, .75, .25], [0., .25, .75]]
+    F[D_FIRST] = [[0., 0., 0.], [0., 1., .75], [0., 0., .25]]
+    F[D_LAST] = [[.25, 0., 0.], [.75, 1., 0.], [0., 0., 0.]]
+    return F
+
+
+def depth_fold_weights(w) -> np.ndarray:
+    return np.einsum("ctk,oiklm->coitlm", depth_fold_matrices(), np.asarray(w, np.float64), optimize=True)
+
+
 def face_delta(p: int, cls: int) -> np.ndarray:
     d = class_matrix(p, cls) - class_matrix(p, INT)
     if cls != INT:
diff --git a/mvs_gi_amd/hip_ops.py b/mvs_gi_amd/hip_ops.py
--- a/mvs_gi_amd/hip_ops.py
+++ b/mvs_gi_amd/hip_ops.py
@@ -11,6 +11,8 @@
 import os
 
 CONV_AUTO, CONV_DIRECT, CONV_MFMA, CONV_BF16X3, CONV_BF16X3_C16, CONV_BF16X3_V32, CONV_BF16X3_D32 = 0, 1, 2, 3, 4, 5, 6
+CONV_BF16X3_UPF_D32 = 8
+CONV_BF16X3_UPF = 7
 SPLIT_F16 = 1
 CONV_F16 = 0x100
 
@@ -368,6 +370,29 @@
     return _pack_bf16(w_oidhw, CONV_BF16X3_C16)
 
 
+def pack_conv_weights_upf(w_oidhw: torch.Tensor, fmt: str = "bf16", layout: int = CONV_BF16X3_UPF):
+    from .dropin.polyphase import depth_fold_weights
+    lib = _lib.load()
+    w = _dev(w_oidhw, "conv weight")
+    Cout, Cin = w.shape[:2]
+    if tuple(w.shape[2:]) != (3, 3, 3) or Cin % 16 or Cout != 32 or (layout == CONV_BF16X3_UPF_D32 and Cin % 32):
+        return None
+    weff = torch.from_numpy(depth_fold_weights(w.detach().cpu().numpy()))
+    unscale = None
+    if fmt == "f16":
+        up, unscale = _pow2_unscale(weff.abs().amax(dim=(0, 2, 3, 4, 5)).float())
+        weff = weff * up.double().view(1, -1, 1, 1, 1, 1)
+        unscale = unscale.to(w.device).contiguous()
+    wf = weff.float().contiguous().to(w.device)
+    wp = torch.empty(lib.mvsgi_conv3d_packed_weight_bytes_upf(Cout, Cin), device=w.device, dtype=torch.uint8)
+    _call("mvsgi_conv3d_pack_weights_split", wf.data_ptr(), wp.data_ptr(), Cout, Cin, layout | (CONV_F16 if _fmt_code(fmt) else 0), _stream_ptr(w))
+    return wp, unscale
+
+
+def conv3d_up2_upf_applies(B, Cin, Dl, Hl, Wl, Cout) -> bool:
+    return bool(_lib.load().mvsgi_conv3d_up2_upf_applies(B, Cin, Dl, Hl, Wl, Cout))
+
+
 def conv3d_d32_applies(B, Cin, Din, Hin, Win, Cout, stride=1) -> bool:
     return bool(_lib.load().mvsgi_conv3d_d32_applies(B, Cin, Din, Hin, Win, Cout, stride))
 
@@ -389,6 +414,8 @@
         return lib.mvsgi_conv3d_packed_weight_bytes_bf16x3_v32(Cout, Cin)
     if layout in (CONV_BF16X3, CONV_BF16X3_D32):
         return lib.mvsgi_conv3d_packed_weight_bytes_bf16x3(Cout, Cin)
+    if layout in (CONV_BF16X3_UPF, CONV_BF16X3_UPF_D32):
+        return lib.mvsgi_conv3d_packed_weight_bytes_upf(Cout, Cin)
     raise ValueError(f"w_layout {layout} is not one of the streaming split kernel's layouts")
 
 
```

Measured after the change: 6355 (median of 6 runs). About the same (+0.7%).
